# osmocom/osmo-trx

Measured on AMD Instinct MI355X. Metric: Mbursts/s detect+demod (156.25 sym, 4 SPS), higher is better.
Workload: dtype f32

## Files before the change

osmo_trx_amd/csrc/trx_kernel_nb.hip:

```cpp
#include "trx_k4_common.h"
#include "trx_nb_asm.inc"

#define NB_D_LEN    160
#define NB_CZ_LEN   (TRX_CZ_PAD + TRX_CORR_NARROW + TRX_CZ_PAD)
#define NB_SLICE    (K4_XS + NB_D_LEN + NB_CZ_LEN)
#define NB_COMP_ROWS (TRX_DELAY_FILTS + 1)
#define NB_TABLES_FLOATS (TRX_SINCV_LDS + 16 * WAVE + NB_COMP_ROWS * 36 + 16 + 8 * 8 + 5 * WAVE + 5 * WAVE + 2 * 8 * 16)
#define NB_TABLES_BYTES (NB_TABLES_FLOATS * 4)
#define NB_WPB 16
#define NB_POOL_RING 64
#define NB_POOL_UNSET (-1)
#define NB_POOL_END (-2)
#define NB_NO_BURST 0xffffffffu
#define NB_LDS_TAIL (16 + 4 * NB_POOL_RING)
#define NB_LDS_BYTES (NB_TABLES_BYTES + NB_WPB * NB_SLICE * 8 + NB_LDS_TAIL)
#define NB_MAX_TOA 32



typedef float v3f __attribute__((ext_vector_type(3)));
typedef int v4i __attribute__((ext_vector_type(4)));

template <typename T>
__device__ __forceinline__ unsigned lds_addr(const T *p)
{
	return (unsigned)(uintptr_t)(const __attribute__((address_space(3))) T *)p;
}

__global__ void __launch_bounds__(NB_WPB * WAVE)
nb_pull4_kernel(const uint32_t *__restrict__ iq, const trxhip_burst_params *__restrict__ params,
		trxhip_burst_result *__restrict__ results, float *__restrict__ soft, const trx_tables *__restrict__ tab,
		unsigned n_bursts, float thresh, float full_scale, unsigned *__restrict__ pool_ctr, unsigned *__restrict__ redo,
		float gk5, float gk6, float gk7, float gk8)
{
	static_assert(NB_TABLES_BYTES % 16 == 0 && (NB_SLICE * 8) % 16 == 0 && (K4_XS * 8) % 16 == 0 && (NB_D_LEN * 8) % 16 == 0, "16-byte LDS accesses");
	static_assert(NB_LDS_BYTES <= 160 * 1024, "LDS");
	static_assert(NB_ASM_GDEC_OFF == (TRX_SINCV_LDS + 16 * WAVE + NB_COMP_ROWS * 36) * 4, "tools/gen_nb_asm.py: LDS offset of the decimator taps");
	static_assert(NB_ASM_DEC_MAX_NACT == 15 + NB_ASM_CORR_MAX_LEN, "tools/gen_nb_asm.py: DEC and CORR change form at the same window");
	static_assert(NB_ASM_LSEQ_OFF == (NB_TABLES_FLOATS - 2 * 8 * 16) * 4, "tools/gen_nb_asm.py: LDS offset of the training-sequence taps");
	constexpr int NLD = 10;
	extern __shared__ __attribute__((aligned(16))) char smem[];
	const int lane0 = threadIdx.x & (WAVE - 1);
	const int wave = uni((int)(threadIdx.x >> 6));

	float *const sincv = reinterpret_cast<float *>(smem);
	float *const wa4f = sincv + TRX_SINCV_LDS;
	const float4 *const wa4 = reinterpret_cast<const float4 *>(wa4f);
	float *const comp = wa4f + 16 * WAVE;
	float *const gdec = comp + NB_COMP_ROWS * 36;
	float *const lhdr = gdec + 16;
	int *const pkcl = reinterpret_cast<int *>(lhdr + 8 * 8);
	int *const lcn = pkcl + 5 * WAVE;
	c32 *const lseq = reinterpret_cast<c32 *>(lcn + 5 * WAVE);
	c32 *const wbase = reinterpret_cast<c32 *>(smem + NB_TABLES_BYTES) + (size_t)wave * NB_SLICE;
	int *const wg_next = reinterpret_cast<int *>(reinterpret_cast<c32 *>(smem + NB_TABLES_BYTES) + (size_t)NB_WPB * NB_SLICE);
	int *const pool_g = wg_next + 4;
	c32 *const P = wbase;
	c32 *const D = wbase + K4_XS;
	c32 *const cz = D + NB_D_LEN + TRX_CZ_PAD;

	for (int i = threadIdx.x; i < TRX_SINCV_LDS; i += blockDim.x)
		sincv[i] = (i < TRX_SINCV_LEN) ? tab->sincv[i] : 0.0f;
	for (int i = threadIdx.x; i < 16 * WAVE; i += blockDim.x) {
		const int l = i & (WAVE - 1), u = i >> 6;
		const PeakConst pcl = peak_const(l);
		const int q = (u < 8) ? pcl.loA + 512 * (7 - u) : pcl.hiA + 512 * (u - 8);
		wa4f[((u >> 2) * WAVE + l) * 4 + (u & 3)] = (q < TRX_SINCV_LEN) ? tab->sincv[q] : 0.0f;
	}
	for (int i = threadIdx.x; i < NB_COMP_ROWS * 36; i += blockDim.x) {
		const int f = i / 36, j = i % 36;
		comp[i] = (j >= TRX_FUSED_SH) ? tab->comp_filt[f][j - TRX_FUSED_SH] : 0.0f;
	}
	if (threadIdx.x < 16)
		gdec[threadIdx.x] = tab->dec_taps[threadIdx.x];
	if (threadIdx.x < 128)
		lseq[threadIdx.x] = make_float2(tab->seq[TRX_SEQ_TSC0 + (threadIdx.x >> 4)].taps[threadIdx.x & 15].re,
						tab->seq[TRX_SEQ_TSC0 + (threadIdx.x >> 4)].taps[threadIdx.x & 15].im);
	if (threadIdx.x < 64)
		lhdr[threadIdx.x] = reinterpret_cast<const float *>(&tab->seq[TRX_SEQ_TSC0 + (threadIdx.x >> 3)].gain)[threadIdx.x & 7];
	if (threadIdx.x < WAVE) {
		const PeakConst pc0 = peak_const(threadIdx.x);
		pkcl[0 * WAVE + threadIdx.x] = pc0.flA;
		pkcl[1 * WAVE + threadIdx.x] = pc0.loA;
		pkcl[2 * WAVE + threadIdx.x] = pc0.hiA;
		pkcl[3 * WAVE + threadIdx.x] = pc0.offB;
		pkcl[4 * WAVE + threadIdx.x] = pc0.ratio_off;
		lcn[0 * WAVE + threadIdx.x] = pc0.ratio_off * 8;
		lcn[1 * WAVE + threadIdx.x] = (pc0.flA - 8) * 8;
		lcn[2 * WAVE + threadIdx.x] = pc0.offB;
		const int l = threadIdx.x, e = (l - 52) / 3, t = (l - 52) % 3;
		const bool sp = l >= 52;
		lcn[3 * WAVE + l] = 8 * (sp ? (t == 0 ? e : t == 1 ? e + 3 : e - 3) : 4 + 3 * (l < 49 ? l : 49));
		lcn[4 * WAVE + l] = sp ? (e + (t == 2 ? 4 : 0)) * K4_NTP * 4 : -1;
	}
	for (int i = lane0; i < NB_SLICE; i += WAVE)
		wbase[i] = make_float2(0.0f, 0.0f);
	if (threadIdx.x == 0) {
		wg_next[0] = NB_WPB;
		wg_next[1] = 0;
	}
	if (threadIdx.x < NB_POOL_RING)
		pool_g[threadIdx.x] = NB_POOL_UNSET;
	__syncthreads();

	const float fs_db = 6.02059991f * __log2f(full_scale);
	const float thr2 = thresh * thresh;
	const float gc0 = thr2 * 1.0001e-5f;
	int t5pk = 0;
	bool t5_ok = true;
	for (int t = 0; t < 8; t++) {
		const int v = (int)(lhdr[8 * t + 5] * 512.0f);
		t5_ok = t5_ok && v >= -8 && v <= 7 && (float)v == lhdr[8 * t + 5] * 512.0f;
		t5pk |= (v & 15) << (4 * t);
	}
	t5pk = uni(t5pk);
	const unsigned long long e8_addr = reinterpret_cast<unsigned long long>(&tab->edge8[0][0][0]);
	const unsigned n_wg = gridDim.x;
	const unsigned n_groups = (n_bursts + 15u) >> 4;
	const bool pooled = pool_ctr != nullptr;
	const unsigned n_static_groups = pooled ? ((n_groups - (n_groups >> 3)) / n_wg) * n_wg : n_groups;
	const unsigned n_pool_groups = n_groups - n_static_groups;
	const unsigned gq = n_static_groups / n_wg, gr = n_static_groups % n_wg;
	const unsigned my_groups = gq + (blockIdx.x < gr ? 1u : 0u);
	const unsigned base16 = (blockIdx.x * gq + (blockIdx.x < gr ? blockIdx.x : gr)) << 4;
	unsigned items = my_groups << 4;
	if (base16 + items > n_bursts)
		items = (base16 < n_bursts) ? n_bursts - base16 : 0u;
	auto burst_of = [&](unsigned jj) -> unsigned {
		if (jj < items)
			return base16 + jj;
		if (!pooled)
			return NB_NO_BURST;
		const unsigned k = (jj - items) >> 4;
		volatile int *slot = pool_g + (k & (NB_POOL_RING - 1));
		int g;
		while ((g = *slot) == NB_POOL_UNSET)
			__builtin_amdgcn_s_sleep(2);
		g = uni(g);
		if (g < 0)
			return NB_NO_BURST;
		const unsigned bb = ((n_static_groups + (unsigned)g) << 4) + (jj & 15u);
		return bb < n_bursts ? bb : NB_NO_BURST;
	};
	auto pool_draw = [&](unsigned jj, bool ended, int lane) {
		const unsigned k = (jj + 16u - items) >> 4;
		int g = NB_POOL_END;
		if (!ended) {
			unsigned p = 0;
			if (lane == 0)
				p = __hip_atomic_fetch_add(pool_ctr, 1u, __ATOMIC_RELAXED, __HIP_MEMORY_SCOPE_AGENT);
			p = (unsigned)uni((int)p);
			g = (p < n_pool_groups) ? (int)p : NB_POOL_END;
		}
		if (lane == 0) {
			pool_g[(k + NB_POOL_RING / 2) & (NB_POOL_RING - 1)] = NB_POOL_UNSET;
			pool_g[k & (NB_POOL_RING - 1)] = g;
		}
	};

	uint32_t pre_i[NLD];
	uint32_t pre_prm = 0u;
	auto prefetch = [&](unsigned bb, int lane) {
		pre_prm = reinterpret_cast<const uint32_t *>(params)[2 * (size_t)bb];
		const uint32_t *src = iq + (size_t)bb * 625;
		const unsigned ul = (unsigned)lane & 63u;
#pragma unroll
		for (int r = 0; r < NLD - 1; r++)
			pre_i[r] = __builtin_nontemporal_load(src + (unsigned)(r * WAVE) + ul);
		pre_i[NLD - 1] = __builtin_nontemporal_load(src + (unsigned)((NLD - 1) * WAVE) + min(ul, 48u));
	};
	const unsigned b_first = burst_of((unsigned)wave);
	if (b_first != NB_NO_BURST)
		prefetch(b_first, lane0);

	v3f o = { 0.0f, 0.0f, 0.0f };
	int recw = 0;
	bool pend_any = false;
	bool pend_rec = false;
	unsigned pend_b = 0;
	bool left_any = false;
	int q_xr = 0, q_xi = 0, q_es = 0, q_toa = 0, q_s = 0, q_fl = 0, q_b = 0;
	int q_n = 0;
	auto flush_records = [&](const int lane) {
		if (lane < q_n) {
			const float *const h = lhdr + 8 * (q_fl & 0xff);
			const float xr = __int_as_float(q_xr), xi = __int_as_float(q_xi);
			const float a0 = xr * h[2], a1 = xr * h[3], a2 = xi * h[3], a3 = xi * h[2];
			const float amp_re = a0 - a2, amp_im = a1 + a3;
			const float toa = (float)q_toa * 0.001953125f;
			const float energy = __int_as_float(q_es) * 0.0125f;
			const float rssi = fs_db - 3.01029996f * __log2f(energy);
			const float p2 = xi * xi + xr * xr;
			const float C = p2 * h[7];
			const float S = __int_as_float(q_s);
			const float ci = 3.0103f * __log2f(C * __builtin_amdgcn_rcpf(S - C));
			const v4i r0 = { 1, __float_as_int(toa), __float_as_int(amp_re), __float_as_int(amp_im) };
			const v4i r1 = { __float_as_int(ci), __float_as_int(energy), __float_as_int(rssi), q_fl };
			asm volatile("global_store_dwordx4 %0, %1, off\n\t"
				     "global_store_dwordx4 %0, %2, off offset:16\n\t"
				     "s_nop 1"
				     :: "v"(results + (unsigned)q_b), "v"(r0), "v"(r1) : "memory");
		}
		q_n = 0;
	};

	auto demod_general = [&](const int nk, const c32 ampv, const int lane) -> bool {
		constexpr int L = 625, nwrite = 148;
		c32 *const dec = D;
		const trx_tables *tabc = tab;
		asm volatile("" : "+s"(tabc));
		const int w = nk >> 7, fr = nk & 127;
		const int fidx = (fr >= 2) ? (fr >> 1) : TRX_DELAY_FILTS;
		const float ian = __builtin_amdgcn_rcpf(norm2(ampv));
		const c32 scale = make_float2(ampv.x * ian, -ampv.y * ian);
		const int n_lo = w > 0 ? w : 0;
		const int n_hi = (L - 1 + w < 623) ? L - 1 + w : 623;
		const int i_full_lo = cdiv4(n_lo + 15), i_full_hi = fdiv4(n_hi);
		const int i0l = cdiv4(n_lo), i0h = i_full_hi + 1;
		const bool need_lo = (n_hi >= n_lo) && (i0l < i_full_lo) && (i0l < nwrite);
		const bool need_hi = (n_hi >= n_lo) && (i0h <= fdiv4(n_hi + 15)) && (i0h < nwrite);
		const bool lo_tab = need_lo && (n_hi >= 4 * (i_full_lo - 1));
		float ct0 = 0.0f, ct1 = 0.0f, ct2 = 0.0f;
		const int le = lane >> 4, lt = lane & 15;
		const int li = i0l + le;
		const int lt0 = n_lo + 15 - 4 * li;
		const bool lact = lt0 >= 1;
		if (lo_tab) {
			const float *row = &tabc->edge_lo[fidx][(lact ? lt0 : 1) - 1][lt];
			ct0 = row[0];
			ct1 = row[16];
			ct2 = (lt < 4) ? row[32] : 0.0f;
		}
		const bool hi_tab = need_hi && (w <= -2) && (n_lo <= 4 * i0h - 15);
		if ((need_lo && !lo_tab) || (need_hi && !hi_tab))
			return false;
		float ch0 = 0.0f, ch1 = 0.0f, ch2 = 0.0f;
		const int hi_i = i0h + le;
		const int htm = n_hi + 15 - 4 * hi_i;
		const bool hact = htm >= 0;
		if (hi_tab) {
			const float *row = &tabc->edge_hi[fidx][hact ? htm : 0][lt];
			ch0 = row[0];
			ch1 = row[16];
			ch2 = (lt < 4) ? row[32] : 0.0f;
		}
		{
			const int c_full = -24 - w;
			const int i_min = cdiv4(-36 - c_full), i_max = fdiv4(L + 1 - c_full);
			int ic = 3 * lane;
			if (ic < i_min) ic = i_min;
			if (ic > i_max - 2) ic = i_max - 2;
			v2f acc[3];
			asm volatile(NB_ASM_FIRG
				     : [a0] "=&v"(acc[0]), [a1] "=&v"(acc[1]), [a2] "=&v"(acc[2])
				     : [nk] "s"(nk), [pb] "s"(lds_addr(P)), [cb] "s"(lds_addr(comp) + 4u * (K4_U0 + TRX_FUSED_SH)), [kic] "v"(8 * ic)
				     : NB_ASM_CLOBBERS);
			if (n_lo == 0 && lo_tab && i_full_hi >= nwrite - 1) {
				if (lane < 52) {
#pragma unroll
					for (int j = 0; j < 3; j++)
						dec[3 * lane + j] = cmul(make_float2(acc[j].x, acc[j].y), scale);
				}
			} else {
#pragma unroll
				for (int j = 0; j < 3; j++) {
					const int i = 3 * lane + j;
					const bool full = (i >= i_full_lo) && (i <= i_full_hi);
					const c32 d = full ? cmul(make_float2(acc[j].x, acc[j].y), scale) : make_float2(0.0f, 0.0f);
					if (i < 156)
						dec[i] = d;
				}
			}
		}
		if (lo_tab) {
			const int s0 = 4 * li - 24 - w + lt;
			const c32 *pp = P + ((s0 & 3) * PH_A + PH_M0 + (s0 >> 2));
			const c32 x0 = lds_c32(pp), x1 = lds_c32(pp + 4), x2 = lds_c32(pp + 8);
			float ar = x0.x * ct0, ai = x0.y * ct0;
			ar = fmaf(x1.x, ct1, ar); ai = fmaf(x1.y, ct1, ai);
			ar = fmaf(x2.x, ct2, ar); ai = fmaf(x2.y, ct2, ai);
			const float sr = row_sum(ar), si = row_sum(ai);
			if (lt == 0 && lact)
				dec[li] = cmul(make_float2(sr, si), scale);
		}
		if (hi_tab) {
			const int s0 = 4 * hi_i - 24 - w + lt;
			const c32 *pp = P + ((s0 & 3) * PH_A + PH_M0 + (s0 >> 2));
			const c32 x0 = lds_c32(pp), x1 = lds_c32(pp + 4), x2 = lds_c32(pp + 8);
			float ar = x0.x * ch0, ai = x0.y * ch0;
			ar = fmaf(x1.x, ch1, ar); ai = fmaf(x1.y, ch1, ai);
			ar = fmaf(x2.x, ch2, ar); ai = fmaf(x2.y, ch2, ai);
			const float sr = row_sum(ar), si = row_sum(ai);
			if (lt == 0 && hact && hi_i < 156)
				dec[hi_i] = cmul(make_float2(sr, si), scale);
		}
		wave_sync();
		auto pick = [&](int i) {
			const float d = reinterpret_cast<const float *>(dec + i)[i & 1];
			return __builtin_amdgcn_fmed3f(fmaf((i & 2) ? -0.5f : 0.5f, d, 0.5f), 0.0f, 1.0f);
		};
		const bool reg = lane >= 2 && lane < 50;
		const int i0 = reg ? 3 * lane - 2 : ((((lane - 54) * 11) >> 5) & 3);
		o.x = pick(i0);
		o.y = pick(reg ? i0 + 1 : 0);
		o.z = pick(reg ? i0 + 2 : 0);
		wave_sync();
		return true;
	};

	DIAG_DECL;
	unsigned j_next = 0, b_next = NB_NO_BURST;
	for (unsigned b = b_first; b != NB_NO_BURST; b = b_next) {
		int lane;
		asm volatile("v_mbcnt_lo_u32_b32 %0, -1, 0\n\tv_mbcnt_hi_u32_b32 %0, -1, %0" : "=v"(lane));
		const int ticket = claim_issue(wg_next);
		const unsigned prm0 = (unsigned)uni((int)pre_prm);
		const unsigned max_toa = prm0 >> 16;
		const int tsc = (prm0 >> 8) & 0xff;
		bool leave = ((prm0 & 0xf8ffu) != (unsigned)TRXHIP_TSC) || (max_toa > NB_MAX_TOA) || !t5_ok;

		c32 *const pload = P + (lane & 3) * PH_A + PH_M0 + (lane >> 2);
		float amax = 0.0f, epart = 0.0f;
#ifdef TRX_DIAG
		DIAG_MARK(12);
		asm volatile("s_waitcnt vmcnt(0)" ::: "memory");
		DIAG_MARK(13);
#endif
		if (!leave) {
#pragma unroll
			for (int r = 0; r < NLD; r++) {
				const int i = r * WAVE + lane;
				if (r < NLD - 1 || i < 625) {
					const c32 v = make_float2((float)(int16_t)(pre_i[r] & 0xffffu), (float)(int16_t)(pre_i[r] >> 16));
					pload[16 * r] = v;
					asm("v_max3_f32 %0, %0, |%1|, |%2|" : "+v"(amax) : "v"(v.x), "v"(v.y));
					if (r < 5)
						epart = fmaf(v.x, v.x, fmaf(v.y, v.y, epart));
				}
			}
		} else {
#pragma unroll
			for (int r = 0; r < NLD; r++)
				asm volatile("" :: "v"(pre_i[r]));
		}
		DIAG_MARK(14);
		if (pend_any) {
			float *const so = soft + (size_t)pend_b * 148;
			int *const rp = reinterpret_cast<int *>(results + pend_b);
			const float oe = o.x;
			asm volatile("s_bfm_b64 exec, 48, 2\n\t"
				     "global_store_dwordx3 %0, %1, %2 offset:16\n\t"
				     "s_mov_b32 exec_lo, 0\n\t"
			     "s_mov_b32 exec_hi, 0x92400000\n\t"
				     "global_store_dword %3, %4, %2\n\t"
				     "s_mov_b64 exec, %8\n\t"
				     "global_store_dword %5, %6, %7\n\t"
				     "s_mov_b64 exec, -1\n\t"
				     "s_nop 0"
				     :: "v"((lane - 2) * 12), "v"(o), "s"(so), "v"((((lane - 54) * 11) >> 5) * 4), "v"(oe), "v"(lane * 4), "v"(recw), "s"(rp),
				        "s"(pend_rec ? 0xffull : 0ull)
				     : "memory");
		}
		pend_any = false;
		DIAG_MARK(16);
		j_next = (unsigned)(leave ? claim_take(ticket) : claim_take_behind<5>(ticket));
		b_next = burst_of(j_next);
		if (pooled && (j_next & 15u) == 0u && j_next + 16u >= items)
			pool_draw(j_next, b_next == NB_NO_BURST && j_next >= items, lane);
		DIAG_MARK(17);
		if (b_next != NB_NO_BURST)
			prefetch(b_next, lane);
		DIAG_MARK(15);

		int clip = 0;
		if (!leave) {
			clip = __ballot(amax > TRX_CLIP_THRESH) != 0ull;

			const int len = 16 + (int)max_toa;
			__builtin_assume(len >= 16 && len <= 16 + NB_MAX_TOA);
			const unsigned vd_addr = lds_addr(D) + 8u * (unsigned)lane, vcz_addr = lds_addr(cz) + 8u * (unsigned)lane;
			unsigned long long bad;
			float dr, di;
			asm volatile(NB_ASM_DEC
				     : [bad] "=s"(bad), [dr] "=&v"(dr), [di] "=&v"(di)
				     : [pd] "v"(lds_addr(P + PH_M0 + 52) + 8u * (unsigned)lane), [vd] "v"(vd_addr), [vd4] "v"(vd_addr - 32u), [zero] "v"(0),
				       [nact] "s"(15 + len)
				     : NB_ASM_CLOBBERS);
			DIAG_MARK(2);
			{
				float v;
				const int lag0 = (len <= NB_ASM_CORR_MAX_LEN) ? NB_ASM_CORR_LANE0 : 0;
				asm volatile(NB_ASM_CORR
					     : [nrm] "=&v"(v)
					     : [vd] "v"(vd_addr), [vcz] "v"(vcz_addr), [vdm] "v"(vd_addr - 8u * NB_ASM_CORR_LANE0),
					       [vczm] "v"(vcz_addr - 8u * NB_ASM_CORR_LANE0), [dr] "v"(dr), [di] "v"(di), [len] "s"(len), [tsc] "s"(tsc), [bad] "s"(bad)
					     : NB_ASM_CLOBBERS);
				DIAG_MARK(3);
				int m_bits, es_bits, bidx;
				int kr, ka, kb, kic, ktp;
				asm volatile(NB_ASM_AMAX("ds_read_b32 %[kr], %[l4] offset:%c[lc]", "ds_read_b32 %[ka], %[l4] offset:%c[lc]+256",
							 "ds_read_b32 %[kb], %[l4] offset:%c[lc]+512", "ds_read_b32 %[kic], %[l4] offset:%c[lc]+768",
							 "ds_read_b32 %[ktp], %[l4] offset:%c[lc]+1024", "s_nop 0", "s_nop 0", "s_nop 0")
					     "s_sub_u32 %[bidx], %[bidx], %[lag0]\n\t"
					     "s_waitcnt lgkmcnt(0)"
					     : [m] "=&s"(m_bits), [es] "=&s"(es_bits), [bidx] "=&s"(bidx), [kr] "=&v"(kr), [ka] "=&v"(ka), [kb] "=&v"(kb),
					       [kic] "=&v"(kic), [ktp] "=&v"(ktp)
					     : [nrm] "v"(v), [ep] "v"(epart), [l4] "v"(4 * lane), [lag0] "s"(lag0),
					       [lc] "n"((TRX_SINCV_LDS + 16 * WAVE + NB_COMP_ROWS * 36 + 16 + 64 + 5 * WAVE) * 4)
					     : NB_ASM_CLOBBERS);
				DIAG_MARK(4);
				int hit = 0;
				int toa512 = 0;
				if (m_bits != 0) {
					int st, e512;
					float km;
					asm volatile(NB_ASM_DETA
						     : [st] "=&s"(st), [e] "=&s"(e512), [km] "=&v"(km)
						     : [bidx] "s"(bidx), [len] "s"(len), [czb] "s"(lds_addr(cz)), [kr] "v"(kr), [ka] "v"(ka), [l16] "v"(16 * lane),
						       [k5] "s"(gk5), [k6] "s"(gk6), [k7] "s"(gk7), [k8] "s"(gk8), [c0] "v"(gc0)
						     : NB_ASM_CLOBBERS);
					DIAG_MARK(5);
					int xr_bits = 0, xi_bits = 0;
					if (st == 1) {
						asm volatile(NB_ASM_DETB
							     : [st] "=&s"(st), [toa] "=&s"(toa512), [xr] "=&s"(xr_bits), [xi] "=&s"(xi_bits)
							     : [e] "s"(e512), [kb] "v"(kb), [czb] "s"(lds_addr(cz)), [km] "v"(km)
							     : NB_ASM_CLOBBERS);
						DIAG_MARK(6);
					}
					if (st == 3) {
						if (lane == 0)
							atomicAdd(&g_trx_fast_stats[0], 1ull);
						PeakConst pkc;
						pkc.flA = pkcl[0 * WAVE + lane]; pkc.loA = pkcl[1 * WAVE + lane]; pkc.hiA = pkcl[2 * WAVE + lane];
						pkc.offB = pkcl[3 * WAVE + lane]; pkc.ratio_off = pkcl[4 * WAVE + lane];
						c32 xcorr;
						peak_detect_spec(cz, bidx, sincv, pkc, lane, &toa512, &xcorr, wa4);
						toa512 = uni(toa512);
						xr_bits = uni(__float_as_int(xcorr.x));
						xi_bits = uni(__float_as_int(xcorr.y));
						st = 1;
					}
					if (st == 2) {
						leave = true;
						if (lane == 0) atomicAdd(&g_trx_fast_stats[2], 1ull);
					}
					if (st == 1) {
						hit = 1;
						int ok, s_bits;
						float d0, d1, d2;
						const int t5 = (t5pk << (28 - 4 * tsc)) >> 28;
						asm volatile("s_setprio 0");
						asm volatile(NB_ASM_TAIL
							     : [ok] "=&s"(ok), [ssum] "=&s"(s_bits), [d0] "=&v"(d0), [d1] "=&v"(d1), [d2] "=&v"(d2)
							     : [toa] "s"(toa512), [xr] "s"(xr_bits), [xi] "s"(xi_bits), [t5] "s"(t5), [hdrb] "s"(lds_addr(lhdr) + 32u * (unsigned)tsc),
							       [e8lo] "s"((unsigned)e8_addr), [e8hi] "s"((unsigned)(e8_addr >> 32)), [l16] "v"(16 * lane),
							       [vd] "v"(vd_addr), [pb] "s"(lds_addr(P)), [cb] "s"(lds_addr(comp) + 4u * (K4_U0 + TRX_FUSED_SH)), [db] "s"(lds_addr(D)),
							       [kic] "v"(kic), [ktp] "v"(ktp)
							     : NB_ASM_CLOBBERS);
						DIAG_MARK(10);
						asm volatile("s_setprio 2");
						if (!ok) {
							if (lane == 0) atomicAdd(&g_trx_fast_stats[3], 1ull);
							const float *const h = lhdr + 8 * tsc;
							const float xr = __int_as_float(xr_bits), xi = __int_as_float(xi_bits);
							const float a0 = xr * h[2], a1 = xr * h[3], a2 = xi * h[3], a3 = xi * h[2];
							const c32 ampv = make_float2(unif(a0 - a2), unif(a1 + a3));
							if (!demod_general(t5 + 10 * 512 - toa512, ampv, lane))
								leave = true;
						}
						if (!leave) {
							asm("s_lshl_b64 exec, 1, %[n]\n\t"
						    "v_mov_b32_e32 %[qxr], %[xr]\n\t"
						    "v_mov_b32_e32 %[qxi], %[xi]\n\t"
						    "v_mov_b32_e32 %[qes], %[es]\n\t"
						    "v_mov_b32_e32 %[qtoa], %[toa]\n\t"
						    "v_mov_b32_e32 %[qs], %[ss]\n\t"
						    "v_mov_b32_e32 %[qfl], %[fl]\n\t"
						    "v_mov_b32_e32 %[qb], %[b]\n\t"
						    "s_mov_b64 exec, -1"
						    : [qxr] "+v"(q_xr), [qxi] "+v"(q_xi), [qes] "+v"(q_es), [qtoa] "+v"(q_toa), [qs] "+v"(q_s), [qfl] "+v"(q_fl),
						      [qb] "+v"(q_b)
						    : [n] "s"(uni(q_n)), [xr] "s"(xr_bits), [xi] "s"(xi_bits), [es] "s"(es_bits), [toa] "s"(toa512 - t5 - 10 * 512),
						      [ss] "s"(s_bits), [fl] "s"((int)((uint32_t)tsc | ((uint32_t)clip << 8) | (37u << 24))), [b] "s"((int)b));
						q_n++;
						}
						if (ok) {
							o.x = __builtin_amdgcn_fmed3f(fmaf(0.5f, d0, 0.5f), 0.0f, 1.0f);
							o.y = __builtin_amdgcn_fmed3f(fmaf(0.5f, d1, 0.5f), 0.0f, 1.0f);
							o.z = __builtin_amdgcn_fmed3f(fmaf(0.5f, d2, 0.5f), 0.0f, 1.0f);
						}
					}
				}
				if (!hit && !leave) {
					const float energy = __int_as_float(es_bits) * 0.0125f;
					const float rssi = fs_db - 3.01029996f * __log2f(energy);
					const uint32_t flags = ((uint32_t)clip << 8) | (1u << 16);
					int word = clip ? -TRXHIP_SIGERR_CLIP : 0;
					word = put_lane<1>(word, 0.0f);
					word = put_lane<2>(word, 0.0f);
					word = put_lane<3>(word, 0.0f);
					word = put_lane<4>(word, 0.0f);
					word = put_lane<5>(word, energy);
					word = put_lane<6>(word, rssi);
					word = write_lane<7>(word, (int)flags);
					recw = word;
					o = (v3f){ 0.0f, 0.0f, 0.0f };
				}
				pend_rec = !hit;
			}
		}
		if (leave) {
			if (lane == 0) {
				reinterpret_cast<uint8_t *>(redo + TRX_REDO_HDR)[b] = 1;
				if (!left_any)
					__hip_atomic_store(redo, 1u, __ATOMIC_RELAXED, __HIP_MEMORY_SCOPE_AGENT);
			}
			left_any = true;
			continue;
		}
		pend_b = b;
		pend_any = true;
		if (q_n == WAVE)
			flush_records(lane);
		DIAG_MARK(11);
	}
	if (pend_any) {
		int lane;
		asm volatile("v_mbcnt_lo_u32_b32 %0, -1, 0\n\tv_mbcnt_hi_u32_b32 %0, -1, %0" : "=v"(lane));
		float *const so = soft + (size_t)pend_b * 148;
		int *const rp = reinterpret_cast<int *>(results + pend_b);
		const float oe = o.x;
		asm volatile("s_bfm_b64 exec, 48, 2\n\t"
			     "global_store_dwordx3 %0, %1, %2 offset:16\n\t"
		     "s_mov_b32 exec_lo, 0\n\t"
		     "s_mov_b32 exec_hi, 0x92400000\n\t"
			     "global_store_dword %3, %4, %2\n\t"
			     "s_mov_b64 exec, %8\n\t"
			     "global_store_dword %5, %6, %7\n\t"
			     "s_mov_b64 exec, -1\n\t"
			     "s_nop 0"
			     :: "v"((lane - 2) * 12), "v"(o), "s"(so), "v"((((lane - 54) * 11) >> 5) * 4), "v"(oe), "v"(lane * 4), "v"(recw), "s"(rp),
			        "s"(pend_rec ? 0xffull : 0ull)
			     : "memory");
	}
	{
		int lane;
		asm volatile("v_mbcnt_lo_u32_b32 %0, -1, 0\n\tv_mbcnt_hi_u32_b32 %0, -1, %0" : "=v"(lane));
		flush_records(lane);
	}
	DIAG_FLUSH();
	if (pooled) {
		__syncthreads();
		int tid0;
		asm volatile("v_mbcnt_lo_u32_b32 %0, -1, 0\n\tv_mbcnt_hi_u32_b32 %0, -1, %0" : "=v"(tid0));
		if (tid0 == 0 && atomicAdd(wg_next + 1, 1) == 0) {
			const unsigned d = __hip_atomic_fetch_add(pool_ctr + 1, 1u, __ATOMIC_ACQ_REL, __HIP_MEMORY_SCOPE_AGENT);
			if (d == gridDim.x - 1u) {
				__hip_atomic_store(pool_ctr, 0u, __ATOMIC_RELAXED, __HIP_MEMORY_SCOPE_AGENT);
				__hip_atomic_store(pool_ctr + 1, 0u, __ATOMIC_RELEASE, __HIP_MEMORY_SCOPE_AGENT);
			}
		}
	}
}
```

osmo_trx_amd/csrc/trx_nb_asm.inc:

```
#define NB_ASM_GDEC_OFF 29968
#define NB_ASM_LSEQ_OFF 32848
#define NB_ASM_DEC_MAX_NACT 60
#define NB_ASM_CORR_LANE0 19
#define NB_ASM_CORR_MAX_LEN 45
#define NB_ASM_CLOBBERS "v64", "v65", "v66", "v67", "v68", "v69", "v70", "v71", "v72", "v73", "v74", "v75", "v76", "v77", "v78", "v79", "v80", "v81", "v82", "v83", "v84", "v85", "v86", "v87", "v88", "v89", "v90", "v91", "v92", "v93", "v94", "v95", "v96", "v97", "v98", "v99", "v100", "v101", "v102", "v103", "v104", "v105", "v106", "v107", "v108", "v109", "v110", "v111", "v112", "v113", "v114", "v115", "v116", "v117", "v118", "v119", "v120", "v121", "v122", "v123", "v124", "v125", "v126", "v127", "s87", "s88", "s89", "s90", "s91", "s92", "s93", "s94", "s95", "s96", "s97", "s98", "s99", "vcc", "scc", "memory"
#define NB_ASM_DEC \
	"s_cmp_gt_u32 %[nact], 60\n\t" \
	"s_cbranch_scc1 .Lnb_dec_wide\n\t" \
	"s_sub_u32 s88, 60, %[nact]\n\t" \
	"s_lshr_b64 exec, -1, s88\n\t" \
	"ds_read_b128 v[120:123], %[zero] offset:29968\n\t" \
	"ds_read_b128 v[124:127], %[zero] offset:29984\n\t" \
	"ds_read_b64 v[98:99], %[pd] offset:1440\n\t" \
	"ds_read_b64 v[100:101], %[pd] offset:2880\n\t" \
	"ds_read_b64 v[102:103], %[pd] offset:4320\n\t" \
	"ds_read_b64 v[96:97], %[pd] offset:0\n\t" \
	"s_waitcnt lgkmcnt(3)\n\t" \
	"v_pk_mul_f32 v[64:65], v[98:99], v[120:121] op_sel:[0,0] op_sel_hi:[1,0]\n\t" \
	"s_waitcnt lgkmcnt(2)\n\t" \
	"v_pk_mul_f32 v[66:67], v[100:101], v[120:121] op_sel:[0,1] op_sel_hi:[1,1]\n\t" \
	"s_waitcnt lgkmcnt(1)\n\t" \
	"v_pk_mul_f32 v[68:69], v[102:103], v[122:123] op_sel:[0,0] op_sel_hi:[1,0]\n\t" \
	"v_pk_add_f32 v[104:105], v[64:65], v[66:67]\n\t" \
	"s_waitcnt lgkmcnt(0)\n\t" \
	"v_pk_mul_f32 v[70:71], v[96:97], v[122:123] op_sel:[0,1] op_sel_hi:[1,1]\n\t" \
	"v_pk_add_f32 v[104:105], v[104:105], v[68:69]\n\t" \
	"v_pk_mul_f32 v[72:73], v[98:99], v[124:125] op_sel:[0,0] op_sel_hi:[1,0]\n\t" \
	"v_pk_mul_f32 v[74:75], v[100:101], v[124:125] op_sel:[0,1] op_sel_hi:[1,1]\n\t" \
	"v_add_f32_dpp v104, v104, v70 wave_shr:1 row_mask:0xf bank_mask:0xf bound_ctrl:0\n\t" \
	"v_add_f32_dpp v105, v105, v71 wave_shr:1 row_mask:0xf bank_mask:0xf bound_ctrl:0\n\t" \
	"v_pk_mul_f32 v[76:77], v[102:103], v[126:127] op_sel:[0,0] op_sel_hi:[1,0]\n\t" \
	"v_pk_add_f32 v[104:105], v[104:105], v[72:73]\n\t" \
	"v_pk_mul_f32 v[78:79], v[96:97], v[126:127] op_sel:[0,1] op_sel_hi:[1,1]\n\t" \
	"v_pk_add_f32 v[104:105], v[104:105], v[74:75]\n\t" \
	"v_pk_mul_f32 v[80:81], v[98:99], v[126:127] op_sel:[0,1] op_sel_hi:[1,1]\n\t" \
	"v_pk_add_f32 v[104:105], v[104:105], v[76:77]\n\t" \
	"v_pk_mul_f32 v[82:83], v[100:101], v[126:127] op_sel:[0,0] op_sel_hi:[1,0]\n\t" \
	"v_pk_mul_f32 v[84:85], v[102:103], v[124:125] op_sel:[0,1] op_sel_hi:[1,1]\n\t" \
	"v_add_f32_dpp v104, v104, v78 wave_shr:1 row_mask:0xf bank_mask:0xf bound_ctrl:0\n\t" \
	"v_add_f32_dpp v105, v105, v79 wave_shr:1 row_mask:0xf bank_mask:0xf bound_ctrl:0\n\t" \
	"v_pk_mul_f32 v[86:87], v[96:97], v[124:125] op_sel:[0,0] op_sel_hi:[1,0]\n\t" \
	"v_pk_add_f32 v[104:105], v[104:105], v[80:81]\n\t" \
	"v_pk_mul_f32 v[88:89], v[98:99], v[122:123] op_sel:[0,1] op_sel_hi:[1,1]\n\t" \
	"v_pk_add_f32 v[104:105], v[104:105], v[82:83]\n\t" \
	"v_pk_mul_f32 v[90:91], v[100:101], v[122:123] op_sel:[0,0] op_sel_hi:[1,0]\n\t" \
	"v_pk_add_f32 v[104:105], v[104:105], v[84:85]\n\t" \
	"v_pk_mul_f32 v[92:93], v[102:103], v[120:121] op_sel:[0,1] op_sel_hi:[1,1]\n\t" \
	"v_pk_mul_f32 v[94:95], v[96:97], v[120:121] op_sel:[0,0] op_sel_hi:[1,0]\n\t" \
	"v_add_f32_dpp v104, v104, v86 wave_shr:1 row_mask:0xf bank_mask:0xf bound_ctrl:0\n\t" \
	"v_add_f32_dpp v105, v105, v87 wave_shr:1 row_mask:0xf bank_mask:0xf bound_ctrl:0\n\t" \
	"v_pk_add_f32 v[104:105], v[104:105], v[88:89]\n\t" \
	"s_nop 0\n\t" \
	"v_pk_add_f32 v[104:105], v[104:105], v[90:91]\n\t" \
	"s_nop 0\n\t" \
	"v_pk_add_f32 v[104:105], v[104:105], v[92:93]\n\t" \
	"s_nop 1\n\t" \
	"v_add_f32_dpp %[dr], v104, v94 wave_shr:1 row_mask:0xf bank_mask:0xf bound_ctrl:0\n\t" \
	"v_add_f32_dpp %[di], v105, v95 wave_shr:1 row_mask:0xf bank_mask:0xf bound_ctrl:0\n\t" \
	"s_bfm_b64 exec, %[nact], 4\n\t" \
	"ds_write2_b32 %[vd4], %[dr], %[di] offset1:1\n\t" \
	"v_min_f32_e64 v106, |%[dr]|, |%[di]|\n\t" \
	"v_max_f32_e64 v107, |%[dr]|, |%[di]|\n\t" \
	"v_ldexp_f32 v106, v106, 17\n\t" \
	"v_cmp_lt_f32_e32 vcc, v106, v107\n\t" \
	"s_mov_b64 exec, -1\n\t" \
	"s_mov_b64 %[bad], vcc\n\t" \
	"s_waitcnt lgkmcnt(0)\n\t" \
	"s_branch .Lnb_dec_end\n\t" \
	".Lnb_dec_wide:\n\t" \
	"s_bfm_b64 exec, %[nact], 0\n\t" \
	"ds_read_b128 v[120:123], %[zero] offset:29968\n\t" \
	"ds_read_b128 v[124:127], %[zero] offset:29984\n\t" \
	"ds_read_b64 v[88:89], %[pd] offset:1440\n\t" \
	"ds_read_b64 v[90:91], %[pd] offset:2880\n\t" \
	"ds_read_b64 v[92:93], %[pd] offset:4320\n\t" \
	"ds_read_b64 v[94:95], %[pd] offset:8\n\t" \
	"ds_read_b64 v[96:97], %[pd] offset:1448\n\t" \
	"ds_read_b64 v[98:99], %[pd] offset:2888\n\t" \
	"ds_read_b64 v[100:101], %[pd] offset:4328\n\t" \
	"ds_read_b64 v[102:103], %[pd] offset:16\n\t" \
	"ds_read_b64 v[104:105], %[pd] offset:1456\n\t" \
	"ds_read_b64 v[106:107], %[pd] offset:2896\n\t" \
	"ds_read_b64 v[108:109], %[pd] offset:4336\n\t" \
	"ds_read_b64 v[110:111], %[pd] offset:24\n\t" \
	"ds_read_b64 v[112:113], %[pd] offset:1464\n\t" \
	"ds_read_b64 v[114:115], %[pd] offset:2904\n\t" \
	"ds_read_b64 v[116:117], %[pd] offset:4344\n\t" \
	"ds_read_b64 v[118:119], %[pd] offset:32\n\t" \
	"s_waitcnt lgkmcnt(12)\n\t" \
	"v_pk_mul_f32 v[88:89], v[88:89], v[120:121] op_sel:[0,0] op_sel_hi:[1,0]\n\t" \
	"v_pk_mul_f32 v[90:91], v[90:91], v[120:121] op_sel:[0,1] op_sel_hi:[1,1]\n\t" \
	"v_pk_mul_f32 v[92:93], v[92:93], v[122:123] op_sel:[0,0] op_sel_hi:[1,0]\n\t" \
	"v_pk_add_f32 v[88:89], v[88:89], v[90:91]\n\t" \
	"v_pk_mul_f32 v[94:95], v[94:95], v[122:123] op_sel:[0,1] op_sel_hi:[1,1]\n\t" \
	"v_pk_add_f32 v[88:89], v[88:89], v[92:93]\n\t" \
	"s_waitcnt lgkmcnt(8)\n\t" \
	"v_pk_mul_f32 v[96:97], v[96:97], v[124:125] op_sel:[0,0] op_sel_hi:[1,0]\n\t" \
	"v_pk_add_f32 v[88:89], v[88:89], v[94:95]\n\t" \
	"v_pk_mul_f32 v[98:99], v[98:99], v[124:125] op_sel:[0,1] op_sel_hi:[1,1]\n\t" \
	"v_pk_add_f32 v[88:89], v[88:89], v[96:97]\n\t" \
	"v_pk_mul_f32 v[100:101], v[100:101], v[126:127] op_sel:[0,0] op_sel_hi:[1,0]\n\t" \
	"v_pk_add_f32 v[88:89], v[88:89], v[98:99]\n\t" \
	"v_pk_mul_f32 v[102:103], v[102:103], v[126:127] op_sel:[0,1] op_sel_hi:[1,1]\n\t" \
	"v_pk_add_f32 v[88:89], v[88:89], v[100:101]\n\t" \
	"s_waitcnt lgkmcnt(4)\n\t" \
	"v_pk_mul_f32 v[104:105], v[104:105], v[126:127] op_sel:[0,1] op_sel_hi:[1,1]\n\t" \
	"v_pk_add_f32 v[88:89], v[88:89], v[102:103]\n\t" \
	"v_pk_mul_f32 v[106:107], v[106:107], v[126:127] op_sel:[0,0] op_sel_hi:[1,0]\n\t" \
	"v_pk_add_f32 v[88:89], v[88:89], v[104:105]\n\t" \
	"v_pk_mul_f32 v[108:109], v[108:109], v[124:125] op_sel:[0,1] op_sel_hi:[1,1]\n\t" \
	"v_pk_add_f32 v[88:89], v[88:89], v[106:107]\n\t" \
	"v_pk_mul_f32 v[110:111], v[110:111], v[124:125] op_sel:[0,0] op_sel_hi:[1,0]\n\t" \
	"v_pk_add_f32 v[88:89], v[88:89], v[108:109]\n\t" \
	"s_waitcnt lgkmcnt(0)\n\t" \
	"v_pk_mul_f32 v[112:113], v[112:113], v[122:123] op_sel:[0,1] op_sel_hi:[1,1]\n\t" \
	"v_pk_add_f32 v[88:89], v[88:89], v[110:111]\n\t" \
	"v_pk_mul_f32 v[114:115], v[114:115], v[122:123] op_sel:[0,0] op_sel_hi:[1,0]\n\t" \
	"v_pk_add_f32 v[88:89], v[88:89], v[112:113]\n\t" \
	"v_pk_mul_f32 v[116:117], v[116:117], v[120:121] op_sel:[0,1] op_sel_hi:[1,1]\n\t" \
	"v_pk_add_f32 v[88:89], v[88:89], v[114:115]\n\t" \
	"v_pk_mul_f32 v[118:119], v[118:119], v[120:121] op_sel:[0,0] op_sel_hi:[1,0]\n\t" \
	"v_pk_add_f32 v[88:89], v[88:89], v[116:117]\n\t" \
	"s_nop 0\n\t" \
	"v_pk_add_f32 v[88:89], v[88:89], v[118:119]\n\t" \
	"ds_write_b64 %[vd], v[88:89]\n\t" \
	"v_min_f32_e64 v90, |v88|, |v89|\n\t" \
	"v_max_f32_e64 v91, |v88|, |v89|\n\t" \
	"v_ldexp_f32 v90, v90, 17\n\t" \
	"v_cmp_lt_f32_e32 vcc, v90, v91\n\t" \
	"s_mov_b64 exec, -1\n\t" \
	"s_mov_b64 %[bad], vcc\n\t" \
	"s_waitcnt lgkmcnt(0)\n\t" \
	".Lnb_dec_end:\n\t"
#define NB_ASM_CORR \
	"s_cmp_gt_u32 %[len], 45\n\t" \
	"s_cbranch_scc1 .Lnb_corr_wide\n\t" \
	"v_mov_b64_e32 v[120:121], 0\n\t" \
	"v_mov_b64_e32 v[122:123], 0\n\t" \
	"v_mov_b32_e32 %[nrm], 0\n\t" \
	"s_lshl_b32 s90, %[len], 3\n\t" \
	"s_sub_u32 s91, 45, %[len]\n\t" \
	"v_add_u32_e32 v64, s90, %[vcz]\n\t" \
	"s_lshr_b64 exec, -1, s91\n\t" \
	"s_cmp_lg_u64 %[bad], 0\n\t" \
	"s_cbranch_scc1 .Lnb_corrr_mul\n\t" \
	"s_getpc_b64 s[88:89]\n\t" \
	".Lnb_corrr_pc:\n\t" \
	"s_mul_i32 s90, %[tsc], .Lnb_corrr_v1-.Lnb_corrr_v0\n\t" \
	"s_add_u32 s88, s88, s90\n\t" \
	"s_addc_u32 s89, s89, 0\n\t" \
	"s_add_u32 s88, s88, .Lnb_corrr_v0-.Lnb_corrr_pc\n\t" \
	"s_addc_u32 s89, s89, 0\n\t" \
	"s_setpc_b64 s[88:89]\n\t" \
	".Lnb_corrr_v0:\n\t" \
	"v_sub_f32_e32 v120, 0, %[dr]\n\t" \
	"v_sub_f32_e32 v121, 0, %[di]\n\t" \
	"s_nop 0\n\t" \
	"v_add_f32_dpp v120, v120, %[di] wave_shr:1 row_mask:0xf bank_mask:0xf bound_ctrl:0\n\t" \
	"v_sub_f32_dpp v121, v121, %[dr] wave_shr:1 row_mask:0xf bank_mask:0xf bound_ctrl:0\n\t" \
	"s_nop 0\n\t" \
	"v_add_f32_dpp v120, v120, %[dr] wave_shr:1 row_mask:0xf bank_mask:0xf bound_ctrl:0\n\t" \
	"v_add_f32_dpp v121, v121, %[di] wave_shr:1 row_mask:0xf bank_mask:0xf bound_ctrl:0\n\t" \
	"s_nop 0\n\t" \
	"v_add_f32_dpp v120, v120, %[di] wave_shr:1 row_mask:0xf bank_mask:0xf bound_ctrl:0\n\t" \
	"v_sub_f32_dpp v121, v121, %[dr] wave_shr:1 row_mask:0xf bank_mask:0xf bound_ctrl:0\n\t" \
	"s_nop 0\n\t" \
	"v_sub_f32_dpp v120, v120, %[dr] wave_shr:1 row_mask:0xf bank_mask:0xf bound_ctrl:0\n\t" \
	"v_sub_f32_dpp v121, v121, %[di] wave_shr:1 row_mask:0xf bank_mask:0xf bound_ctrl:0\n\t" \
	"s_nop 0\n\t" \
	"v_add_f32_dpp v120, v120, %[di] wave_shr:1 row_mask:0xf bank_mask:0xf bound_ctrl:0\n\t" \
	"v_sub_f32_dpp v121, v121, %[dr] wave_shr:1 row_mask:0xf bank_mask:0xf bound_ctrl:0\n\t" \
	"s_nop 0\n\t" \
	"v_sub_f32_dpp v120, v120, %[dr] wave_shr:1 row_mask:0xf bank_mask:0xf bound_ctrl:0\n\t" \
	"v_sub_f32_dpp v121, v121, %[di] wave_shr:1 row_mask:0xf bank_mask:0xf bound_ctrl:0\n\t" \
	"s_nop 0\n\t" \
	"v_sub_f32_dpp v120, v120, %[di] wave_shr:1 row_mask:0xf bank_mask:0xf bound_ctrl:0\n\t" \
	"v_add_f32_dpp v121, v121, %[dr] wave_shr:1 row_mask:0xf bank_mask:0xf bound_ctrl:0\n\t" \
	"s_nop 0\n\t" \
	"v_add_f32_dpp v120, v120, %[dr] wave_shr:1 row_mask:0xf bank_mask:0xf bound_ctrl:0\n\t" \
	"v_add_f32_dpp v121, v121, %[di] wave_shr:1 row_mask:0xf bank_mask:0xf bound_ctrl:0\n\t" \
	"s_nop 0\n\t" \
	"v_sub_f32_dpp v120, v120, %[di] wave_shr:1 row_mask:0xf bank_mask:0xf bound_ctrl:0\n\t" \
	"v_add_f32_dpp v121, v121, %[dr] wave_shr:1 row_mask:0xf bank_mask:0xf bound_ctrl:0\n\t" \
	"s_nop 0\n\t" \
	"v_sub_f32_dpp v120, v120, %[dr] wave_shr:1 row_mask:0xf bank_mask:0xf bound_ctrl:0\n\t" \
	"v_sub_f32_dpp v121, v121, %[di] wave_shr:1 row_mask:0xf bank_mask:0xf bound_ctrl:0\n\t" \
	"s_nop 0\n\t" \
	"v_sub_f32_dpp v120, v120, %[di] wave_shr:1 row_mask:0xf bank_mask:0xf bound_ctrl:0\n\t" \
	"v_add_f32_dpp v121, v121, %[dr] wave_shr:1 row_mask:0xf bank_mask:0xf bound_ctrl:0\n\t" \
	"s_nop 0\n\t" \
	"v_add_f32_dpp v120, v120, %[dr] wave_shr:1 row_mask:0xf bank_mask:0xf bound_ctrl:0\n\t" \
	"v_add_f32_dpp v121, v121, %[di] wave_shr:1 row_mask:0xf bank_mask:0xf bound_ctrl:0\n\t" \
	"s_nop 0\n\t" \
	"v_sub_f32_dpp v120, v120, %[di] wave_shr:1 row_mask:0xf bank_mask:0xf bound_ctrl:0\n\t" \
	"v_add_f32_dpp v121, v121, %[dr] wave_shr:1 row_mask:0xf bank_mask:0xf bound_ctrl:0\n\t" \
	"s_nop 0\n\t" \
	"v_sub_f32_dpp v120, v120, %[dr] wave_shr:1 row_mask:0xf bank_mask:0xf bound_ctrl:0\n\t" \
	"v_sub_f32_dpp v121, v121, %[di] wave_shr:1 row_mask:0xf bank_mask:0xf bound_ctrl:0\n\t" \
	"s_nop 0\n\t" \
	"v_sub_f32_dpp v120, v120, %[di] wave_shr:1 row_mask:0xf bank_mask:0xf bound_ctrl:0\n\t" \
	"v_add_f32_dpp v121, v121, %[dr] wave_shr:1 row_mask:0xf bank_mask:0xf bound_ctrl:0\n\t" \
	"s_branch .Lnb_corrr_join\n\t" \
	".Lnb_corrr_v1:\n\t" \
	"v_sub_f32_e32 v120, 0, %[dr]\n\t" \
	"v_sub_f32_e32 v121, 0, %[di]\n\t" \
	"s_nop 0\n\t" \
	"v_add_f32_dpp v120, v120, %[di] wave_shr:1 row_mask:0xf bank_mask:0xf bound_ctrl:0\n\t" \
	"v_sub_f32_dpp v121, v121, %[dr] wave_shr:1 row_mask:0xf bank_mask:0xf bound_ctrl:0\n\t" \
	"s_nop 0\n\t" \
	"v_add_f32_dpp v120, v120, %[dr] wave_shr:1 row_mask:0xf bank_mask:0xf bound_ctrl:0\n\t" \
	"v_add_f32_dpp v121, v121, %[di] wave_shr:1 row_mask:0xf bank_mask:0xf bound_ctrl:0\n\t" \
	"s_nop 0\n\t" \
	"v_add_f32_dpp v120, v120, %[di] wave_shr:1 row_mask:0xf bank_mask:0xf bound_ctrl:0\n\t" \
	"v_sub_f32_dpp v121, v121, %[dr] wave_shr:1 row_mask:0xf bank_mask:0xf bound_ctrl:0\n\t" \
	"s_nop 0\n\t" \
	"v_sub_f32_dpp v120, v120, %[dr] wave_shr:1 row_mask:0xf bank_mask:0xf bound_ctrl:0\n\t" \
	"v_sub_f32_dpp v121, v121, %[di] wave_shr:1 row_mask:0xf bank_mask:0xf bound_ctrl:0\n\t" \
	"s_nop 0\n\t" \
	"v_add_f32_dpp v120, v120, %[di] wave_shr:1 row_mask:0xf bank_mask:0xf bound_ctrl:0\n\t" \
	"v_sub_f32_dpp v121, v121, %[dr] wave_shr:1 row_mask:0xf bank_mask:0xf bound_ctrl:0\n\t" \
	"s_nop 0\n\t" \
	"v_add_f32_dpp v120, v120, %[dr] wave_shr:1 row_mask:0xf bank_mask:0xf bound_ctrl:0\n\t" \
	"v_add_f32_dpp v121, v121, %[di] wave_shr:1 row_mask:0xf bank_mask:0xf bound_ctrl:0\n\t" \
	"s_nop 0\n\t" \
	"v_add_f32_dpp v120, v120, %[di] wave_shr:1 row_mask:0xf bank_mask:0xf bound_ctrl:0\n\t" \
	"v_sub_f32_dpp v121, v121, %[dr] wave_shr:1 row_mask:0xf bank_mask:0xf bound_ctrl:0\n\t" \
	"s_nop 0\n\t" \
	"v_sub_f32_dpp v120, v120, %[dr] wave_shr:1 row_mask:0xf bank_mask:0xf bound_ctrl:0\n\t" \
	"v_sub_f32_dpp v121, v121, %[di] wave_shr:1 row_mask:0xf bank_mask:0xf bound_ctrl:0\n\t" \
	"s_nop 0\n\t" \
	"v_sub_f32_dpp v120, v120, %[di] wave_shr:1 row_mask:0xf bank_mask:0xf bound_ctrl:0\n\t" \
	"v_add_f32_dpp v121, v121, %[dr] wave_shr:1 row_mask:0xf bank_mask:0xf bound_ctrl:0\n\t" \
	"s_nop 0\n\t" \
	"v_sub_f32_dpp v120, v120, %[dr] wave_shr:1 row_mask:0xf bank_mask:0xf bound_ctrl:0\n\t" \
	"v_sub_f32_dpp v121, v121, %[di] wave_shr:1 row_mask:0xf bank_mask:0xf bound_ctrl:0\n\t" \
	"s_nop 0\n\t" \
	"v_sub_f32_dpp v120, v120, %[di] wave_shr:1 row_mask:0xf bank_mask:0xf bound_ctrl:0\n\t" \
	"v_add_f32_dpp v121, v121, %[dr] wave_shr:1 row_mask:0xf bank_mask:0xf bound_ctrl:0\n\t" \
	"s_nop 0\n\t" \
	"v_add_f32_dpp v120, v120, %[dr] wave_shr:1 row_mask:0xf bank_mask:0xf bound_ctrl:0\n\t" \
	"v_add_f32_dpp v121, v121, %[di] wave_shr:1 row_mask:0xf bank_mask:0xf bound_ctrl:0\n\t" \
	"s_nop 0\n\t" \
	"v_sub_f32_dpp v120, v120, %[di] wave_shr:1 row_mask:0xf bank_mask:0xf bound_ctrl:0\n\t" \
	"v_add_f32_dpp v121, v121, %[dr] wave_shr:1 row_mask:0xf bank_mask:0xf bound_ctrl:0\n\t" \
	"s_nop 0\n\t" \
	"v_sub_f32_dpp v120, v120, %[dr] wave_shr:1 row_mask:0xf bank_mask:0xf bound_ctrl:0\n\t" \
	"v_sub_f32_dpp v121, v121, %[di] wave_shr:1 row_mask:0xf bank_mask:0xf bound_ctrl:0\n\t" \
	"s_nop 0\n\t" \
	"v_add_f32_dpp v120, v120, %[di] wave_shr:1 row_mask:0xf bank_mask:0xf bound_ctrl:0\n\t" \
	"v_sub_f32_dpp v121, v121, %[dr] wave_shr:1 row_mask:0xf bank_mask:0xf bound_ctrl:0\n\t" \
	"s_branch .Lnb_corrr_join\n\t" \
	".Lnb_corrr_v2:\n\t" \
	"v_add_f32_e32 v120, 0, %[dr]\n\t" \
	"v_add_f32_e32 v121, 0, %[di]\n\t" \
	"s_nop 0\n\t" \
	"v_sub_f32_dpp v120, v120, %[di] wave_shr:1 row_mask:0xf bank_mask:0xf bound_ctrl:0\n\t" \
	"v_add_f32_dpp v121, v121, %[dr] wave_shr:1 row_mask:0xf bank_mask:0xf bound_ctrl:0\n\t" \
	"s_nop 0\n\t" \
	"v_add_f32_dpp v120, v120, %[dr] wave_shr:1 row_mask:0xf bank_mask:0xf bound_ctrl:0\n\t" \
	"v_add_f32_dpp v121, v121, %[di] wave_shr:1 row_mask:0xf bank_mask:0xf bound_ctrl:0\n\t" \
	"s_nop 0\n\t" \
	"v_add_f32_dpp v120, v120, %[di] wave_shr:1 row_mask:0xf bank_mask:0xf bound_ctrl:0\n\t" \
	"v_sub_f32_dpp v121, v121, %[dr] wave_shr:1 row_mask:0xf bank_mask:0xf bound_ctrl:0\n\t" \
	"s_nop 0\n\t" \
	"v_add_f32_dpp v120, v120, %[dr] wave_shr:1 row_mask:0xf bank_mask:0xf bound_ctrl:0\n\t" \
	"v_add_f32_dpp v121, v121, %[di] wave_shr:1 row_mask:0xf bank_mask:0xf bound_ctrl:0\n\t" \
	"s_nop 0\n\t" \
	"v_sub_f32_dpp v120, v120, %[di] wave_shr:1 row_mask:0xf bank_mask:0xf bound_ctrl:0\n\t" \
	"v_add_f32_dpp v121, v121, %[dr] wave_shr:1 row_mask:0xf bank_mask:0xf bound_ctrl:0\n\t" \
	"s_nop 0\n\t" \
	"v_add_f32_dpp v120, v120, %[dr] wave_shr:1 row_mask:0xf bank_mask:0xf bound_ctrl:0\n\t" \
	"v_add_f32_dpp v121, v121, %[di] wave_shr:1 row_mask:0xf bank_mask:0xf bound_ctrl:0\n\t" \
	"s_nop 0\n\t" \
	"v_add_f32_dpp v120, v120, %[di] wave_shr:1 row_mask:0xf bank_mask:0xf bound_ctrl:0\n\t" \
	"v_sub_f32_dpp v121, v121, %[dr] wave_shr:1 row_mask:0xf bank_mask:0xf bound_ctrl:0\n\t" \
	"s_nop 0\n\t" \
	"v_add_f32_dpp v120, v120, %[dr] wave_shr:1 row_mask:0xf bank_mask:0xf bound_ctrl:0\n\t" \
	"v_add_f32_dpp v121, v121, %[di] wave_shr:1 row_mask:0xf bank_mask:0xf bound_ctrl:0\n\t" \
	"s_nop 0\n\t" \
	"v_sub_f32_dpp v120, v120, %[di] wave_shr:1 row_mask:0xf bank_mask:0xf bound_ctrl:0\n\t" \
	"v_add_f32_dpp v121, v121, %[dr] wave_shr:1 row_mask:0xf bank_mask:0xf bound_ctrl:0\n\t" \
	"s_nop 0\n\t" \
	"v_sub_f32_dpp v120, v120, %[dr] wave_shr:1 row_mask:0xf bank_mask:0xf bound_ctrl:0\n\t" \
	"v_sub_f32_dpp v121, v121, %[di] wave_shr:1 row_mask:0xf bank_mask:0xf bound_ctrl:0\n\t" \
	"s_nop 0\n\t" \
	"v_sub_f32_dpp v120, v120, %[di] wave_shr:1 row_mask:0xf bank_mask:0xf bound_ctrl:0\n\t" \
	"v_add_f32_dpp v121, v121, %[dr] wave_shr:1 row_mask:0xf bank_mask:0xf bound_ctrl:0\n\t" \
	"s_nop 0\n\t" \
	"v_sub_f32_dpp v120, v120, %[dr] wave_shr:1 row_mask:0xf bank_mask:0xf bound_ctrl:0\n\t" \
	"v_sub_f32_dpp v121, v121, %[di] wave_shr:1 row_mask:0xf bank_mask:0xf bound_ctrl:0\n\t" \
	"s_nop 0\n\t" \
	"v_add_f32_dpp v120, v120, %[di] wave_shr:1 row_mask:0xf bank_mask:0xf bound_ctrl:0\n\t" \
	"v_sub_f32_dpp v121, v121, %[dr] wave_shr:1 row_mask:0xf bank_mask:0xf bound_ctrl:0\n\t" \
	"s_nop 0\n\t" \
	"v_sub_f32_dpp v120, v120, %[dr] wave_shr:1 row_mask:0xf bank_mask:0xf bound_ctrl:0\n\t" \
	"v_sub_f32_dpp v121, v121, %[di] wave_shr:1 row_mask:0xf bank_mask:0xf bound_ctrl:0\n\t" \
	"s_nop 0\n\t" \
	"v_sub_f32_dpp v120, v120, %[di] wave_shr:1 row_mask:0xf bank_mask:0xf bound_ctrl:0\n\t" \
	"v_add_f32_dpp v121, v121, %[dr] wave_shr:1 row_mask:0xf bank_mask:0xf bound_ctrl:0\n\t" \
	"s_branch .Lnb_corrr_join\n\t" \
	".Lnb_corrr_v3:\n\t" \
	"v_sub_f32_e32 v120, 0, %[dr]\n\t" \
	"v_sub_f32_e32 v121, 0, %[di]\n\t" \
	"s_nop 0\n\t" \
	"v_sub_f32_dpp v120, v120, %[di] wave_shr:1 row_mask:0xf bank_mask:0xf bound_ctrl:0\n\t" \
	"v_add_f32_dpp v121, v121, %[dr] wave_shr:1 row_mask:0xf bank_mask:0xf bound_ctrl:0\n\t" \
	"s_nop 0\n\t" \
// ... 494 lines not shown
	"s_waitcnt lgkmcnt(5)\n\t" \
	"v_pk_add_f32 v[120:121], v[120:121], v[108:109] neg_lo:[0,1] neg_hi:[0,1]\n\t" \
	"s_waitcnt lgkmcnt(4)\n\t" \
	"v_pk_add_f32 v[120:121], v[120:121], v[110:111] op_sel:[0,1] op_sel_hi:[1,0] neg_lo:[0,1] neg_hi:[0,0]\n\t" \
	"s_waitcnt lgkmcnt(3)\n\t" \
	"v_pk_add_f32 v[120:121], v[120:121], v[112:113] neg_lo:[0,1] neg_hi:[0,1]\n\t" \
	"s_waitcnt lgkmcnt(2)\n\t" \
	"v_pk_add_f32 v[120:121], v[120:121], v[114:115] op_sel:[0,1] op_sel_hi:[1,0] neg_lo:[0,0] neg_hi:[0,1]\n\t" \
	"s_waitcnt lgkmcnt(1)\n\t" \
	"v_pk_add_f32 v[120:121], v[120:121], v[116:117] neg_lo:[0,1] neg_hi:[0,1]\n\t" \
	"s_waitcnt lgkmcnt(0)\n\t" \
	"v_pk_add_f32 v[120:121], v[120:121], v[118:119] op_sel:[0,1] op_sel_hi:[1,0] neg_lo:[0,1] neg_hi:[0,0]\n\t" \
	"s_branch .Lnb_corrw_join\n\t" \
	".Lnb_corrw_v3:\n\t" \
	"s_waitcnt lgkmcnt(15)\n\t" \
	"v_pk_add_f32 v[120:121], v[120:121], v[88:89] neg_lo:[0,1] neg_hi:[0,1]\n\t" \
	"s_waitcnt lgkmcnt(14)\n\t" \
	"v_pk_add_f32 v[120:121], v[120:121], v[90:91] op_sel:[0,1] op_sel_hi:[1,0] neg_lo:[0,1] neg_hi:[0,0]\n\t" \
	"s_waitcnt lgkmcnt(13)\n\t" \
	"v_pk_add_f32 v[120:121], v[120:121], v[92:93]\n\t" \
	"s_waitcnt lgkmcnt(12)\n\t" \
	"v_pk_add_f32 v[120:121], v[120:121], v[94:95] op_sel:[0,1] op_sel_hi:[1,0] neg_lo:[0,0] neg_hi:[0,1]\n\t" \
	"s_waitcnt lgkmcnt(11)\n\t" \
	"v_pk_add_f32 v[120:121], v[120:121], v[96:97]\n\t" \
	"s_waitcnt lgkmcnt(10)\n\t" \
	"v_pk_add_f32 v[120:121], v[120:121], v[98:99] op_sel:[0,1] op_sel_hi:[1,0] neg_lo:[0,1] neg_hi:[0,0]\n\t" \
	"s_waitcnt lgkmcnt(9)\n\t" \
	"v_pk_add_f32 v[120:121], v[120:121], v[100:101]\n\t" \
	"s_waitcnt lgkmcnt(8)\n\t" \
	"v_pk_add_f32 v[120:121], v[120:121], v[102:103] op_sel:[0,1] op_sel_hi:[1,0] neg_lo:[0,1] neg_hi:[0,0]\n\t" \
	"s_waitcnt lgkmcnt(7)\n\t" \
	"v_pk_add_f32 v[120:121], v[120:121], v[104:105] neg_lo:[0,1] neg_hi:[0,1]\n\t" \
	"s_waitcnt lgkmcnt(6)\n\t" \
	"v_pk_add_f32 v[120:121], v[120:121], v[106:107] op_sel:[0,1] op_sel_hi:[1,0] neg_lo:[0,0] neg_hi:[0,1]\n\t" \
	"s_waitcnt lgkmcnt(5)\n\t" \
	"v_pk_add_f32 v[120:121], v[120:121], v[108:109] neg_lo:[0,1] neg_hi:[0,1]\n\t" \
	"s_waitcnt lgkmcnt(4)\n\t" \
	"v_pk_add_f32 v[120:121], v[120:121], v[110:111] op_sel:[0,1] op_sel_hi:[1,0] neg_lo:[0,1] neg_hi:[0,0]\n\t" \
	"s_waitcnt lgkmcnt(3)\n\t" \
	"v_pk_add_f32 v[120:121], v[120:121], v[112:113] neg_lo:[0,1] neg_hi:[0,1]\n\t" \
	"s_waitcnt lgkmcnt(2)\n\t" \
	"v_pk_add_f32 v[120:121], v[120:121], v[114:115] op_sel:[0,1] op_sel_hi:[1,0] neg_lo:[0,0] neg_hi:[0,1]\n\t" \
	"s_waitcnt lgkmcnt(1)\n\t" \
	"v_pk_add_f32 v[120:121], v[120:121], v[116:117] neg_lo:[0,1] neg_hi:[0,1]\n\t" \
	"s_waitcnt lgkmcnt(0)\n\t" \
	"v_pk_add_f32 v[120:121], v[120:121], v[118:119] op_sel:[0,1] op_sel_hi:[1,0] neg_lo:[0,1] neg_hi:[0,0]\n\t" \
	"s_branch .Lnb_corrw_join\n\t" \
	".Lnb_corrw_v4:\n\t" \
	"s_waitcnt lgkmcnt(15)\n\t" \
	"v_pk_add_f32 v[120:121], v[120:121], v[88:89]\n\t" \
	"s_waitcnt lgkmcnt(14)\n\t" \
	"v_pk_add_f32 v[120:121], v[120:121], v[90:91] op_sel:[0,1] op_sel_hi:[1,0] neg_lo:[0,1] neg_hi:[0,0]\n\t" \
	"s_waitcnt lgkmcnt(13)\n\t" \
	"v_pk_add_f32 v[120:121], v[120:121], v[92:93] neg_lo:[0,1] neg_hi:[0,1]\n\t" \
	"s_waitcnt lgkmcnt(12)\n\t" \
	"v_pk_add_f32 v[120:121], v[120:121], v[94:95] op_sel:[0,1] op_sel_hi:[1,0] neg_lo:[0,0] neg_hi:[0,1]\n\t" \
	"s_waitcnt lgkmcnt(11)\n\t" \
	"v_pk_add_f32 v[120:121], v[120:121], v[96:97] neg_lo:[0,1] neg_hi:[0,1]\n\t" \
	"s_waitcnt lgkmcnt(10)\n\t" \
	"v_pk_add_f32 v[120:121], v[120:121], v[98:99] op_sel:[0,1] op_sel_hi:[1,0] neg_lo:[0,1] neg_hi:[0,0]\n\t" \
	"s_waitcnt lgkmcnt(9)\n\t" \
	"v_pk_add_f32 v[120:121], v[120:121], v[100:101] neg_lo:[0,1] neg_hi:[0,1]\n\t" \
	"s_waitcnt lgkmcnt(8)\n\t" \
	"v_pk_add_f32 v[120:121], v[120:121], v[102:103] op_sel:[0,1] op_sel_hi:[1,0] neg_lo:[0,1] neg_hi:[0,0]\n\t" \
	"s_waitcnt lgkmcnt(7)\n\t" \
	"v_pk_add_f32 v[120:121], v[120:121], v[104:105] neg_lo:[0,1] neg_hi:[0,1]\n\t" \
	"s_waitcnt lgkmcnt(6)\n\t" \
	"v_pk_add_f32 v[120:121], v[120:121], v[106:107] op_sel:[0,1] op_sel_hi:[1,0] neg_lo:[0,0] neg_hi:[0,1]\n\t" \
	"s_waitcnt lgkmcnt(5)\n\t" \
	"v_pk_add_f32 v[120:121], v[120:121], v[108:109] neg_lo:[0,1] neg_hi:[0,1]\n\t" \
	"s_waitcnt lgkmcnt(4)\n\t" \
	"v_pk_add_f32 v[120:121], v[120:121], v[110:111] op_sel:[0,1] op_sel_hi:[1,0] neg_lo:[0,1] neg_hi:[0,0]\n\t" \
	"s_waitcnt lgkmcnt(3)\n\t" \
	"v_pk_add_f32 v[120:121], v[120:121], v[112:113]\n\t" \
	"s_waitcnt lgkmcnt(2)\n\t" \
	"v_pk_add_f32 v[120:121], v[120:121], v[114:115] op_sel:[0,1] op_sel_hi:[1,0] neg_lo:[0,0] neg_hi:[0,1]\n\t" \
	"s_waitcnt lgkmcnt(1)\n\t" \
	"v_pk_add_f32 v[120:121], v[120:121], v[116:117]\n\t" \
	"s_waitcnt lgkmcnt(0)\n\t" \
	"v_pk_add_f32 v[120:121], v[120:121], v[118:119] op_sel:[0,1] op_sel_hi:[1,0] neg_lo:[0,0] neg_hi:[0,1]\n\t" \
	"s_branch .Lnb_corrw_join\n\t" \
	".Lnb_corrw_v5:\n\t" \
	"s_waitcnt lgkmcnt(15)\n\t" \
	"v_pk_add_f32 v[120:121], v[120:121], v[88:89] neg_lo:[0,1] neg_hi:[0,1]\n\t" \
	"s_waitcnt lgkmcnt(14)\n\t" \
	"v_pk_add_f32 v[120:121], v[120:121], v[90:91] op_sel:[0,1] op_sel_hi:[1,0] neg_lo:[0,1] neg_hi:[0,0]\n\t" \
	"s_waitcnt lgkmcnt(13)\n\t" \
	"v_pk_add_f32 v[120:121], v[120:121], v[92:93] neg_lo:[0,1] neg_hi:[0,1]\n\t" \
	"s_waitcnt lgkmcnt(12)\n\t" \
	"v_pk_add_f32 v[120:121], v[120:121], v[94:95] op_sel:[0,1] op_sel_hi:[1,0] neg_lo:[0,0] neg_hi:[0,1]\n\t" \
	"s_waitcnt lgkmcnt(11)\n\t" \
	"v_pk_add_f32 v[120:121], v[120:121], v[96:97]\n\t" \
	"s_waitcnt lgkmcnt(10)\n\t" \
	"v_pk_add_f32 v[120:121], v[120:121], v[98:99] op_sel:[0,1] op_sel_hi:[1,0] neg_lo:[0,1] neg_hi:[0,0]\n\t" \
	"s_waitcnt lgkmcnt(9)\n\t" \
	"v_pk_add_f32 v[120:121], v[120:121], v[100:101]\n\t" \
	"s_waitcnt lgkmcnt(8)\n\t" \
	"v_pk_add_f32 v[120:121], v[120:121], v[102:103] op_sel:[0,1] op_sel_hi:[1,0] neg_lo:[0,1] neg_hi:[0,0]\n\t" \
	"s_waitcnt lgkmcnt(7)\n\t" \
	"v_pk_add_f32 v[120:121], v[120:121], v[104:105]\n\t" \
	"s_waitcnt lgkmcnt(6)\n\t" \
	"v_pk_add_f32 v[120:121], v[120:121], v[106:107] op_sel:[0,1] op_sel_hi:[1,0] neg_lo:[0,0] neg_hi:[0,1]\n\t" \
	"s_waitcnt lgkmcnt(5)\n\t" \
	"v_pk_add_f32 v[120:121], v[120:121], v[108:109] neg_lo:[0,1] neg_hi:[0,1]\n\t" \
	"s_waitcnt lgkmcnt(4)\n\t" \
	"v_pk_add_f32 v[120:121], v[120:121], v[110:111] op_sel:[0,1] op_sel_hi:[1,0] neg_lo:[0,1] neg_hi:[0,0]\n\t" \
	"s_waitcnt lgkmcnt(3)\n\t" \
	"v_pk_add_f32 v[120:121], v[120:121], v[112:113] neg_lo:[0,1] neg_hi:[0,1]\n\t" \
	"s_waitcnt lgkmcnt(2)\n\t" \
	"v_pk_add_f32 v[120:121], v[120:121], v[114:115] op_sel:[0,1] op_sel_hi:[1,0] neg_lo:[0,0] neg_hi:[0,1]\n\t" \
	"s_waitcnt lgkmcnt(1)\n\t" \
	"v_pk_add_f32 v[120:121], v[120:121], v[116:117] neg_lo:[0,1] neg_hi:[0,1]\n\t" \
	"s_waitcnt lgkmcnt(0)\n\t" \
	"v_pk_add_f32 v[120:121], v[120:121], v[118:119] op_sel:[0,1] op_sel_hi:[1,0] neg_lo:[0,0] neg_hi:[0,1]\n\t" \
	"s_branch .Lnb_corrw_join\n\t" \
	".Lnb_corrw_v6:\n\t" \
	"s_waitcnt lgkmcnt(15)\n\t" \
	"v_pk_add_f32 v[120:121], v[120:121], v[88:89] neg_lo:[0,1] neg_hi:[0,1]\n\t" \
	"s_waitcnt lgkmcnt(14)\n\t" \
	"v_pk_add_f32 v[120:121], v[120:121], v[90:91] op_sel:[0,1] op_sel_hi:[1,0] neg_lo:[0,1] neg_hi:[0,0]\n\t" \
	"s_waitcnt lgkmcnt(13)\n\t" \
	"v_pk_add_f32 v[120:121], v[120:121], v[92:93]\n\t" \
	"s_waitcnt lgkmcnt(12)\n\t" \
	"v_pk_add_f32 v[120:121], v[120:121], v[94:95] op_sel:[0,1] op_sel_hi:[1,0] neg_lo:[0,0] neg_hi:[0,1]\n\t" \
	"s_waitcnt lgkmcnt(11)\n\t" \
	"v_pk_add_f32 v[120:121], v[120:121], v[96:97] neg_lo:[0,1] neg_hi:[0,1]\n\t" \
	"s_waitcnt lgkmcnt(10)\n\t" \
	"v_pk_add_f32 v[120:121], v[120:121], v[98:99] op_sel:[0,1] op_sel_hi:[1,0] neg_lo:[0,0] neg_hi:[0,1]\n\t" \
	"s_waitcnt lgkmcnt(9)\n\t" \
	"v_pk_add_f32 v[120:121], v[120:121], v[100:101]\n\t" \
	"s_waitcnt lgkmcnt(8)\n\t" \
	"v_pk_add_f32 v[120:121], v[120:121], v[102:103] op_sel:[0,1] op_sel_hi:[1,0] neg_lo:[0,0] neg_hi:[0,1]\n\t" \
	"s_waitcnt lgkmcnt(7)\n\t" \
	"v_pk_add_f32 v[120:121], v[120:121], v[104:105]\n\t" \
	"s_waitcnt lgkmcnt(6)\n\t" \
	"v_pk_add_f32 v[120:121], v[120:121], v[106:107] op_sel:[0,1] op_sel_hi:[1,0] neg_lo:[0,0] neg_hi:[0,1]\n\t" \
	"s_waitcnt lgkmcnt(5)\n\t" \
	"v_pk_add_f32 v[120:121], v[120:121], v[108:109] neg_lo:[0,1] neg_hi:[0,1]\n\t" \
	"s_waitcnt lgkmcnt(4)\n\t" \
	"v_pk_add_f32 v[120:121], v[120:121], v[110:111] op_sel:[0,1] op_sel_hi:[1,0] neg_lo:[0,0] neg_hi:[0,1]\n\t" \
	"s_waitcnt lgkmcnt(3)\n\t" \
	"v_pk_add_f32 v[120:121], v[120:121], v[112:113]\n\t" \
	"s_waitcnt lgkmcnt(2)\n\t" \
	"v_pk_add_f32 v[120:121], v[120:121], v[114:115] op_sel:[0,1] op_sel_hi:[1,0] neg_lo:[0,1] neg_hi:[0,0]\n\t" \
	"s_waitcnt lgkmcnt(1)\n\t" \
	"v_pk_add_f32 v[120:121], v[120:121], v[116:117] neg_lo:[0,1] neg_hi:[0,1]\n\t" \
	"s_waitcnt lgkmcnt(0)\n\t" \
	"v_pk_add_f32 v[120:121], v[120:121], v[118:119] op_sel:[0,1] op_sel_hi:[1,0] neg_lo:[0,1] neg_hi:[0,0]\n\t" \
	"s_branch .Lnb_corrw_join\n\t" \
	".Lnb_corrw_v7:\n\t" \
	"s_waitcnt lgkmcnt(15)\n\t" \
	"v_pk_add_f32 v[120:121], v[120:121], v[88:89] neg_lo:[0,1] neg_hi:[0,1]\n\t" \
	"s_waitcnt lgkmcnt(14)\n\t" \
	"v_pk_add_f32 v[120:121], v[120:121], v[90:91] op_sel:[0,1] op_sel_hi:[1,0] neg_lo:[0,1] neg_hi:[0,0]\n\t" \
	"s_waitcnt lgkmcnt(13)\n\t" \
	"v_pk_add_f32 v[120:121], v[120:121], v[92:93]\n\t" \
	"s_waitcnt lgkmcnt(12)\n\t" \
	"v_pk_add_f32 v[120:121], v[120:121], v[94:95] op_sel:[0,1] op_sel_hi:[1,0] neg_lo:[0,1] neg_hi:[0,0]\n\t" \
	"s_waitcnt lgkmcnt(11)\n\t" \
	"v_pk_add_f32 v[120:121], v[120:121], v[96:97]\n\t" \
	"s_waitcnt lgkmcnt(10)\n\t" \
	"v_pk_add_f32 v[120:121], v[120:121], v[98:99] op_sel:[0,1] op_sel_hi:[1,0] neg_lo:[0,0] neg_hi:[0,1]\n\t" \
	"s_waitcnt lgkmcnt(9)\n\t" \
	"v_pk_add_f32 v[120:121], v[120:121], v[100:101]\n\t" \
	"s_waitcnt lgkmcnt(8)\n\t" \
	"v_pk_add_f32 v[120:121], v[120:121], v[102:103] op_sel:[0,1] op_sel_hi:[1,0] neg_lo:[0,1] neg_hi:[0,0]\n\t" \
	"s_waitcnt lgkmcnt(7)\n\t" \
	"v_pk_add_f32 v[120:121], v[120:121], v[104:105]\n\t" \
	"s_waitcnt lgkmcnt(6)\n\t" \
	"v_pk_add_f32 v[120:121], v[120:121], v[106:107] op_sel:[0,1] op_sel_hi:[1,0] neg_lo:[0,1] neg_hi:[0,0]\n\t" \
	"s_waitcnt lgkmcnt(5)\n\t" \
	"v_pk_add_f32 v[120:121], v[120:121], v[108:109] neg_lo:[0,1] neg_hi:[0,1]\n\t" \
	"s_waitcnt lgkmcnt(4)\n\t" \
	"v_pk_add_f32 v[120:121], v[120:121], v[110:111] op_sel:[0,1] op_sel_hi:[1,0] neg_lo:[0,0] neg_hi:[0,1]\n\t" \
	"s_waitcnt lgkmcnt(3)\n\t" \
	"v_pk_add_f32 v[120:121], v[120:121], v[112:113] neg_lo:[0,1] neg_hi:[0,1]\n\t" \
	"s_waitcnt lgkmcnt(2)\n\t" \
	"v_pk_add_f32 v[120:121], v[120:121], v[114:115] op_sel:[0,1] op_sel_hi:[1,0] neg_lo:[0,1] neg_hi:[0,0]\n\t" \
	"s_waitcnt lgkmcnt(1)\n\t" \
	"v_pk_add_f32 v[120:121], v[120:121], v[116:117] neg_lo:[0,1] neg_hi:[0,1]\n\t" \
	"s_waitcnt lgkmcnt(0)\n\t" \
	"v_pk_add_f32 v[120:121], v[120:121], v[118:119] op_sel:[0,1] op_sel_hi:[1,0] neg_lo:[0,0] neg_hi:[0,1]\n\t" \
	"s_branch .Lnb_corrw_join\n\t" \
	".Lnb_corrw_join:\n\t" \
	"s_add_u32 s90, %[len], 12\n\t" \
	"s_bfm_b64 exec, s90, 0\n\t" \
	"ds_write_b64 %[vcz], v[120:121]\n\t" \
	"s_mov_b64 exec, -1\n\t" \
	"v_pk_mul_f32 v[122:123], v[120:121], v[120:121]\n\t" \
	"s_waitcnt lgkmcnt(0)\n\t" \
	"v_add_f32_e32 %[nrm], v123, v122\n\t" \
	"s_branch .Lnb_corr_end\n\t" \
	".Lnb_corrw_mul:\n\t" \
	"s_lshl_b32 s90, %[tsc], 7\n\t" \
	"v_mov_b32_e32 v64, s90\n\t" \
	"ds_read_b128 v[66:69], v64 offset:32848\n\t" \
	"ds_read_b128 v[70:73], v64 offset:32864\n\t" \
	"ds_read_b128 v[74:77], v64 offset:32880\n\t" \
	"ds_read_b128 v[78:81], v64 offset:32896\n\t" \
	"s_waitcnt lgkmcnt(0)\n\t" \
	"v_pk_mul_f32 v[82:83], v[88:89], v[66:67] op_sel:[0,0] op_sel_hi:[0,1]\n\t" \
	"v_pk_mul_f32 v[84:85], v[88:89], v[66:67] op_sel:[1,1] op_sel_hi:[1,0]\n\t" \
	"s_nop 0\n\t" \
	"v_pk_add_f32 v[86:87], v[82:83], v[84:85] neg_lo:[0,1] neg_hi:[0,0]\n\t" \
	"s_nop 0\n\t" \
	"v_pk_add_f32 v[120:121], v[120:121], v[86:87]\n\t" \
	"v_pk_mul_f32 v[82:83], v[90:91], v[68:69] op_sel:[0,0] op_sel_hi:[0,1]\n\t" \
	"v_pk_mul_f32 v[84:85], v[90:91], v[68:69] op_sel:[1,1] op_sel_hi:[1,0]\n\t" \
	"s_nop 0\n\t" \
	"v_pk_add_f32 v[86:87], v[82:83], v[84:85] neg_lo:[0,1] neg_hi:[0,0]\n\t" \
	"s_nop 0\n\t" \
	"v_pk_add_f32 v[120:121], v[120:121], v[86:87]\n\t" \
	"v_pk_mul_f32 v[82:83], v[92:93], v[70:71] op_sel:[0,0] op_sel_hi:[0,1]\n\t" \
	"v_pk_mul_f32 v[84:85], v[92:93], v[70:71] op_sel:[1,1] op_sel_hi:[1,0]\n\t" \
	"s_nop 0\n\t" \
	"v_pk_add_f32 v[86:87], v[82:83], v[84:85] neg_lo:[0,1] neg_hi:[0,0]\n\t" \
	"s_nop 0\n\t" \
	"v_pk_add_f32 v[120:121], v[120:121], v[86:87]\n\t" \
	"v_pk_mul_f32 v[82:83], v[94:95], v[72:73] op_sel:[0,0] op_sel_hi:[0,1]\n\t" \
	"v_pk_mul_f32 v[84:85], v[94:95], v[72:73] op_sel:[1,1] op_sel_hi:[1,0]\n\t" \
	"s_nop 0\n\t" \
	"v_pk_add_f32 v[86:87], v[82:83], v[84:85] neg_lo:[0,1] neg_hi:[0,0]\n\t" \
	"s_nop 0\n\t" \
	"v_pk_add_f32 v[120:121], v[120:121], v[86:87]\n\t" \
	"v_pk_mul_f32 v[82:83], v[96:97], v[74:75] op_sel:[0,0] op_sel_hi:[0,1]\n\t" \
	"v_pk_mul_f32 v[84:85], v[96:97], v[74:75] op_sel:[1,1] op_sel_hi:[1,0]\n\t" \
	"s_nop 0\n\t" \
	"v_pk_add_f32 v[86:87], v[82:83], v[84:85] neg_lo:[0,1] neg_hi:[0,0]\n\t" \
	"s_nop 0\n\t" \
	"v_pk_add_f32 v[120:121], v[120:121], v[86:87]\n\t" \
	"v_pk_mul_f32 v[82:83], v[98:99], v[76:77] op_sel:[0,0] op_sel_hi:[0,1]\n\t" \
	"v_pk_mul_f32 v[84:85], v[98:99], v[76:77] op_sel:[1,1] op_sel_hi:[1,0]\n\t" \
	"s_nop 0\n\t" \
	"v_pk_add_f32 v[86:87], v[82:83], v[84:85] neg_lo:[0,1] neg_hi:[0,0]\n\t" \
	"s_nop 0\n\t" \
	"v_pk_add_f32 v[120:121], v[120:121], v[86:87]\n\t" \
	"v_pk_mul_f32 v[82:83], v[100:101], v[78:79] op_sel:[0,0] op_sel_hi:[0,1]\n\t" \
	"v_pk_mul_f32 v[84:85], v[100:101], v[78:79] op_sel:[1,1] op_sel_hi:[1,0]\n\t" \
	"s_nop 0\n\t" \
	"v_pk_add_f32 v[86:87], v[82:83], v[84:85] neg_lo:[0,1] neg_hi:[0,0]\n\t" \
	"s_nop 0\n\t" \
	"v_pk_add_f32 v[120:121], v[120:121], v[86:87]\n\t" \
	"v_pk_mul_f32 v[82:83], v[102:103], v[80:81] op_sel:[0,0] op_sel_hi:[0,1]\n\t" \
	"v_pk_mul_f32 v[84:85], v[102:103], v[80:81] op_sel:[1,1] op_sel_hi:[1,0]\n\t" \
	"s_nop 0\n\t" \
	"v_pk_add_f32 v[86:87], v[82:83], v[84:85] neg_lo:[0,1] neg_hi:[0,0]\n\t" \
	"s_nop 0\n\t" \
	"v_pk_add_f32 v[120:121], v[120:121], v[86:87]\n\t" \
	"ds_read_b128 v[66:69], v64 offset:32912\n\t" \
	"ds_read_b128 v[70:73], v64 offset:32928\n\t" \
	"ds_read_b128 v[74:77], v64 offset:32944\n\t" \
	"ds_read_b128 v[78:81], v64 offset:32960\n\t" \
	"s_waitcnt lgkmcnt(0)\n\t" \
	"v_pk_mul_f32 v[82:83], v[104:105], v[66:67] op_sel:[0,0] op_sel_hi:[0,1]\n\t" \
	"v_pk_mul_f32 v[84:85], v[104:105], v[66:67] op_sel:[1,1] op_sel_hi:[1,0]\n\t" \
	"s_nop 0\n\t" \
	"v_pk_add_f32 v[86:87], v[82:83], v[84:85] neg_lo:[0,1] neg_hi:[0,0]\n\t" \
	"s_nop 0\n\t" \
	"v_pk_add_f32 v[120:121], v[120:121], v[86:87]\n\t" \
	"v_pk_mul_f32 v[82:83], v[106:107], v[68:69] op_sel:[0,0] op_sel_hi:[0,1]\n\t" \
	"v_pk_mul_f32 v[84:85], v[106:107], v[68:69] op_sel:[1,1] op_sel_hi:[1,0]\n\t" \
	"s_nop 0\n\t" \
	"v_pk_add_f32 v[86:87], v[82:83], v[84:85] neg_lo:[0,1] neg_hi:[0,0]\n\t" \
	"s_nop 0\n\t" \
	"v_pk_add_f32 v[120:121], v[120:121], v[86:87]\n\t" \
	"v_pk_mul_f32 v[82:83], v[108:109], v[70:71] op_sel:[0,0] op_sel_hi:[0,1]\n\t" \
	"v_pk_mul_f32 v[84:85], v[108:109], v[70:71] op_sel:[1,1] op_sel_hi:[1,0]\n\t" \
	"s_nop 0\n\t" \
	"v_pk_add_f32 v[86:87], v[82:83], v[84:85] neg_lo:[0,1] neg_hi:[0,0]\n\t" \
	"s_nop 0\n\t" \
	"v_pk_add_f32 v[120:121], v[120:121], v[86:87]\n\t" \
	"v_pk_mul_f32 v[82:83], v[110:111], v[72:73] op_sel:[0,0] op_sel_hi:[0,1]\n\t" \
	"v_pk_mul_f32 v[84:85], v[110:111], v[72:73] op_sel:[1,1] op_sel_hi:[1,0]\n\t" \
	"s_nop 0\n\t" \
	"v_pk_add_f32 v[86:87], v[82:83], v[84:85] neg_lo:[0,1] neg_hi:[0,0]\n\t" \
	"s_nop 0\n\t" \
	"v_pk_add_f32 v[120:121], v[120:121], v[86:87]\n\t" \
	"v_pk_mul_f32 v[82:83], v[112:113], v[74:75] op_sel:[0,0] op_sel_hi:[0,1]\n\t" \
	"v_pk_mul_f32 v[84:85], v[112:113], v[74:75] op_sel:[1,1] op_sel_hi:[1,0]\n\t" \
	"s_nop 0\n\t" \
	"v_pk_add_f32 v[86:87], v[82:83], v[84:85] neg_lo:[0,1] neg_hi:[0,0]\n\t" \
	"s_nop 0\n\t" \
	"v_pk_add_f32 v[120:121], v[120:121], v[86:87]\n\t" \
	"v_pk_mul_f32 v[82:83], v[114:115], v[76:77] op_sel:[0,0] op_sel_hi:[0,1]\n\t" \
	"v_pk_mul_f32 v[84:85], v[114:115], v[76:77] op_sel:[1,1] op_sel_hi:[1,0]\n\t" \
	"s_nop 0\n\t" \
	"v_pk_add_f32 v[86:87], v[82:83], v[84:85] neg_lo:[0,1] neg_hi:[0,0]\n\t" \
	"s_nop 0\n\t" \
	"v_pk_add_f32 v[120:121], v[120:121], v[86:87]\n\t" \
	"v_pk_mul_f32 v[82:83], v[116:117], v[78:79] op_sel:[0,0] op_sel_hi:[0,1]\n\t" \
	"v_pk_mul_f32 v[84:85], v[116:117], v[78:79] op_sel:[1,1] op_sel_hi:[1,0]\n\t" \
	"s_nop 0\n\t" \
	"v_pk_add_f32 v[86:87], v[82:83], v[84:85] neg_lo:[0,1] neg_hi:[0,0]\n\t" \
	"s_nop 0\n\t" \
	"v_pk_add_f32 v[120:121], v[120:121], v[86:87]\n\t" \
	"v_pk_mul_f32 v[82:83], v[118:119], v[80:81] op_sel:[0,0] op_sel_hi:[0,1]\n\t" \
	"v_pk_mul_f32 v[84:85], v[118:119], v[80:81] op_sel:[1,1] op_sel_hi:[1,0]\n\t" \
	"s_nop 0\n\t" \
	"v_pk_add_f32 v[86:87], v[82:83], v[84:85] neg_lo:[0,1] neg_hi:[0,0]\n\t" \
	"s_nop 0\n\t" \
	"v_pk_add_f32 v[120:121], v[120:121], v[86:87]\n\t" \
	"s_branch .Lnb_corrw_join\n\t" \
	".Lnb_corr_end:\n\t"
#define NB_ASM_DETA \
	"s_mov_b32 %[st], 0\n\t" \
	"s_cmp_lt_i32 %[bidx], 3\n\t" \
	"s_cbranch_scc1 .Lnb_da_end\n\t" \
	"s_sub_u32 s88, %[len], 3\n\t" \
	"s_cmp_gt_i32 %[bidx], s88\n\t" \
	"s_cbranch_scc1 .Lnb_da_end\n\t" \
	"s_lshl3_add_u32 s89, %[bidx], %[czb]\n\t" \
	"s_add_u32 s90, %[len], -1\n\t" \
	"v_mov_b32_e32 v64, s89\n\t" \
	"v_add_u32_e32 v65, s89, %[kr]\n\t" \
	"s_lshl3_add_u32 s90, s90, %[czb]\n\t" \
	"v_add_u32_e32 v66, s89, %[ka]\n\t" \
	"ds_read_b64 v[68:69], v64\n\t" \
	"v_mov_b32_e32 v67, s90\n\t" \
	"v_mov_b64_e32 v[72:73], 0\n\t" \
	"s_bfm_b64 exec, 8, 0\n\t" \
	"ds_read_b64 v[70:71], v65\n\t" \
	"s_mov_b64 exec, 1\n\t" \
	"ds_write_b64 v67, v[72:73]\n\t" \
	"s_mov_b64 exec, -1\n\t" \
	"ds_read_b128 v[76:79], %[l16] offset:16512\n\t" \
	"ds_read_b128 v[80:83], %[l16] offset:17536\n\t" \
	"ds_read_b64 v[88:89], v66 offset:0\n\t" \
	"ds_read_b64 v[90:91], v66 offset:8\n\t" \
	"ds_read_b64 v[92:93], v66 offset:16\n\t" \
	"ds_read_b64 v[94:95], v66 offset:24\n\t" \
	"ds_read_b64 v[96:97], v66 offset:32\n\t" \
	"ds_read_b64 v[98:99], v66 offset:40\n\t" \
	"ds_read_b64 v[100:101], v66 offset:48\n\t" \
	"ds_read_b64 v[102:103], v66 offset:56\n\t" \
	"v_mov_b64_e32 v[84:85], 0\n\t" \
	"v_mov_b64_e32 v[86:87], 0\n\t" \
	"s_add_u32 s91, %[bidx], -1\n\t" \
	"s_sub_u32 s92, %[len], %[bidx]\n\t" \
	"s_min_u32 s91, s91, 4\n\t" \
	"s_waitcnt lgkmcnt(11)\n\t" \
	"v_pk_mul_f32 v[68:69], v[68:69], v[68:69]\n\t" \
	"s_add_u32 s92, s92, -2\n\t" \
	"v_add_f32_e32 v74, v69, v68\n\t" \
	"v_mul_f32_e32 %[km], 0x36c9539c, v74\n\t" \
	"s_bfm_b64 exec, 8, 0\n\t" \
	"v_pk_mul_f32 v[70:71], v[70:71], v[70:71]\n\t" \
	"s_min_u32 s92, s92, 4\n\t" \
	"v_add_f32_e32 v75, v71, v70\n\t" \
	"s_add_u32 s91, s91, s92\n\t" \
	"s_cmp_eq_u32 s91, 8\n\t" \
	"v_add_f32_dpp v75, v75, v75 quad_perm:[1,0,3,2] row_mask:0xf bank_mask:0xf\n\t" \
	"s_cselect_b32 s92, %[k8], %[k7]\n\t" \
	"s_cmp_eq_u32 s91, 6\n\t" \
	"v_add_f32_dpp v75, v75, v75 quad_perm:[2,3,0,1] row_mask:0xf bank_mask:0xf\n\t" \
	"s_cselect_b32 s93, %[k6], %[k5]\n\t" \
	"s_cmp_ge_u32 s91, 7\n\t" \
	"v_add_f32_dpp v75, v75, v75 row_half_mirror row_mask:0xf bank_mask:0xf\n\t" \
	"s_cselect_b32 s92, s92, s93\n\t" \
	"v_mul_f32_e32 v112, s92, v75\n\t" \
	"v_mul_f32_e32 v113, 0x3f7fff37, v112\n\t" \
	"v_fmamk_f32 v114, v112, 0x3f8000c9, %[c0]\n\t" \
	"v_cmp_lt_f32_e32 vcc, v74, v113\n\t" \
	"s_cbranch_vccnz .Lnb_da_wait_end\n\t" \
	"v_cmp_gt_f32_e32 vcc, v74, v114\n\t" \
	"s_mov_b32 %[st], 2\n\t" \
	"s_cbranch_vccz .Lnb_da_wait_end\n\t" \
	"s_mov_b64 exec, -1\n\t" \
	"ds_read_b128 v[104:107], %[l16] offset:18560\n\t" \
	"ds_read_b128 v[108:111], %[l16] offset:19584\n\t" \
	"ds_read_b64 v[112:113], v66 offset:64\n\t" \
	"ds_read_b64 v[114:115], v66 offset:72\n\t" \
	"ds_read_b64 v[116:117], v66 offset:80\n\t" \
	"ds_read_b64 v[118:119], v66 offset:88\n\t" \
	"ds_read_b64 v[120:121], v66 offset:96\n\t" \
	"ds_read_b64 v[122:123], v66 offset:104\n\t" \
	"ds_read_b64 v[124:125], v66 offset:112\n\t" \
	"ds_read_b64 v[126:127], v66 offset:120\n\t" \
	"s_waitcnt lgkmcnt(10)\n\t" \
	"v_pk_fma_f32 v[84:85], v[88:89], v[76:77], v[84:85] op_sel:[0,0,0] op_sel_hi:[1,0,1]\n\t" \
	"v_pk_fma_f32 v[86:87], v[90:91], v[76:77], v[86:87] op_sel:[0,1,0] op_sel_hi:[1,1,1]\n\t" \
	"v_pk_fma_f32 v[84:85], v[92:93], v[78:79], v[84:85] op_sel:[0,0,0] op_sel_hi:[1,0,1]\n\t" \
	"v_pk_fma_f32 v[86:87], v[94:95], v[78:79], v[86:87] op_sel:[0,1,0] op_sel_hi:[1,1,1]\n\t" \
	"v_pk_fma_f32 v[84:85], v[96:97], v[80:81], v[84:85] op_sel:[0,0,0] op_sel_hi:[1,0,1]\n\t" \
	"v_pk_fma_f32 v[86:87], v[98:99], v[80:81], v[86:87] op_sel:[0,1,0] op_sel_hi:[1,1,1]\n\t" \
	"v_pk_fma_f32 v[84:85], v[100:101], v[82:83], v[84:85] op_sel:[0,0,0] op_sel_hi:[1,0,1]\n\t" \
	"v_pk_fma_f32 v[86:87], v[102:103], v[82:83], v[86:87] op_sel:[0,1,0] op_sel_hi:[1,1,1]\n\t" \
	"s_waitcnt lgkmcnt(0)\n\t" \
	"v_pk_fma_f32 v[84:85], v[112:113], v[104:105], v[84:85] op_sel:[0,0,0] op_sel_hi:[1,0,1]\n\t" \
	"v_pk_fma_f32 v[86:87], v[114:115], v[104:105], v[86:87] op_sel:[0,1,0] op_sel_hi:[1,1,1]\n\t" \
	"v_pk_fma_f32 v[84:85], v[116:117], v[106:107], v[84:85] op_sel:[0,0,0] op_sel_hi:[1,0,1]\n\t" \
	"v_pk_fma_f32 v[86:87], v[118:119], v[106:107], v[86:87] op_sel:[0,1,0] op_sel_hi:[1,1,1]\n\t" \
	"v_pk_fma_f32 v[84:85], v[120:121], v[108:109], v[84:85] op_sel:[0,0,0] op_sel_hi:[1,0,1]\n\t" \
	"v_pk_fma_f32 v[86:87], v[122:123], v[108:109], v[86:87] op_sel:[0,1,0] op_sel_hi:[1,1,1]\n\t" \
	"v_pk_fma_f32 v[84:85], v[124:125], v[110:111], v[84:85] op_sel:[0,0,0] op_sel_hi:[1,0,1]\n\t" \
	"v_pk_fma_f32 v[86:87], v[126:127], v[110:111], v[86:87] op_sel:[0,1,0] op_sel_hi:[1,1,1]\n\t" \
	"s_nop 0\n\t" \
	"v_pk_add_f32 v[84:85], v[84:85], v[86:87]\n\t" \
	"s_nop 0\n\t" \
	"v_pk_mul_f32 v[84:85], v[84:85], v[84:85]\n\t" \
	"s_nop 0\n\t" \
	"v_add_f32_e32 v88, v85, v84\n\t" \
	"v_fmamk_f32 v89, v88, 0x36c9539c, %[km]\n\t" \
	"v_sub_f32_e32 v90, v88, v89\n\t" \
	"v_add_f32_e32 v91, v88, v89\n\t" \
	"s_lshl_b32 s94, %[bidx], 9\n\t" \
	"v_mov_b32_dpp v90, v90 quad_perm:[1,0,3,2] row_mask:0xf bank_mask:0xf\n\t" \
	"v_cmp_lt_f32_e64 s[88:89], v91, v90\n\t" \
	"s_mov_b32 %[st], 1\n\t" \
	"s_lshr_b64 s[90:91], s[88:89], 1\n\t" \
	"s_or_b64 s[90:91], s[90:91], s[88:89]\n\t" \
	"s_mov_b32 s96, 0x55555555\n\t" \
	"s_mov_b32 s97, 0x15555555\n\t" \
	"s_and_b64 s[92:93], s[90:91], s[96:97]\n\t" \
	"s_cmp_eq_u64 s[92:93], s[96:97]\n\t" \
	"s_cbranch_scc0 .Lnb_da_careful\n\t" \
	"s_mov_b32 s95, 0\n\t" \
	"s_lshl1_add_u32 s96, s95, 0\n\t" \
	"s_bitcmp1_b64 s[88:89], s96\n\t" \
	"s_addc_u32 s95, s95, s95\n\t" \
	"s_lshl1_add_u32 s96, s95, 2\n\t" \
	"s_bitcmp1_b64 s[88:89], s96\n\t" \
	"s_addc_u32 s95, s95, s95\n\t" \
	"s_lshl1_add_u32 s96, s95, 6\n\t" \
	"s_bitcmp1_b64 s[88:89], s96\n\t" \
	"s_addc_u32 s95, s95, s95\n\t" \
	"s_lshl1_add_u32 s96, s95, 14\n\t" \
	"s_bitcmp1_b64 s[88:89], s96\n\t" \
	"s_addc_u32 s95, s95, s95\n\t" \
	"s_lshl1_add_u32 s96, s95, 30\n\t" \
	"s_bitcmp1_b64 s[88:89], s96\n\t" \
	"s_addc_u32 s95, s95, s95\n\t" \
	".Lnb_da_walked:\n\t" \
	"s_lshl_b32 s95, s95, 5\n\t" \
	"s_add_u32 s94, s94, s95\n\t" \
	"s_add_u32 %[e], s94, -1008\n\t" \
	"s_branch .Lnb_da_end\n\t" \
	".Lnb_da_careful:\n\t" \
	"s_mov_b32 s95, 0\n\t" \
	"s_lshl1_add_u32 s96, s95, 0\n\t" \
	"s_bitcmp0_b64 s[90:91], s96\n\t" \
	"s_cbranch_scc1 .Lnb_da_unsure\n\t" \
	"s_bitcmp1_b64 s[88:89], s96\n\t" \
	"s_addc_u32 s95, s95, s95\n\t" \
	"s_lshl1_add_u32 s96, s95, 2\n\t" \
	"s_bitcmp0_b64 s[90:91], s96\n\t" \
	"s_cbranch_scc1 .Lnb_da_unsure\n\t" \
	"s_bitcmp1_b64 s[88:89], s96\n\t" \
	"s_addc_u32 s95, s95, s95\n\t" \
	"s_lshl1_add_u32 s96, s95, 6\n\t" \
	"s_bitcmp0_b64 s[90:91], s96\n\t" \
	"s_cbranch_scc1 .Lnb_da_unsure\n\t" \
	"s_bitcmp1_b64 s[88:89], s96\n\t" \
	"s_addc_u32 s95, s95, s95\n\t" \
	"s_lshl1_add_u32 s96, s95, 14\n\t" \
	"s_bitcmp0_b64 s[90:91], s96\n\t" \
	"s_cbranch_scc1 .Lnb_da_unsure\n\t" \
	"s_bitcmp1_b64 s[88:89], s96\n\t" \
	"s_addc_u32 s95, s95, s95\n\t" \
	"s_lshl1_add_u32 s96, s95, 30\n\t" \
	"s_bitcmp0_b64 s[90:91], s96\n\t" \
	"s_cbranch_scc1 .Lnb_da_unsure\n\t" \
	"s_bitcmp1_b64 s[88:89], s96\n\t" \
	"s_addc_u32 s95, s95, s95\n\t" \
	"s_branch .Lnb_da_walked\n\t" \
	".Lnb_da_unsure:\n\t" \
	"s_mov_b32 %[st], 3\n\t" \
	"s_branch .Lnb_da_end\n\t" \
	".Lnb_da_wait_end:\n\t" \
	"s_mov_b64 exec, -1\n\t" \
	"s_waitcnt lgkmcnt(0)\n\t" \
	".Lnb_da_end:\n\t"
#define NB_ASM_DETB \
	"v_mov_b64_e32 v[64:65], 0\n\t" \
	"v_mov_b64_e32 v[66:67], 0\n\t" \
	"v_add_u32_e32 v68, %[e], %[kb]\n\t" \
	"s_add_u32 s88, %[czb], -56\n\t" \
	"s_mov_b32 exec_lo, 0x3fffffff\n\t" \
	"s_mov_b32 exec_hi, 0xffff\n\t" \
	"v_ashrrev_i32_e32 v69, 9, v68\n\t" \
	"v_and_b32_e32 v70, 0x1ff, v68\n\t" \
	"v_lshl_add_u32 v69, v69, 3, s88\n\t" \
	"v_bfe_u32 v71, v70, 4, 5\n\t" \
	"v_sub_u32_e32 v72, 0x200, v70\n\t" \
	"v_xor_b32_e32 v71, v71, v70\n\t" \
	"v_bfe_u32 v73, v72, 4, 5\n\t" \
	"v_lshlrev_b32_e32 v71, 2, v71\n\t" \
	"v_xor_b32_e32 v72, v73, v72\n\t" \
	"v_lshlrev_b32_e32 v72, 2, v72\n\t" \
	"ds_read_b64 v[80:81], v69 offset:0\n\t" \
	"ds_read_b32 v96, v71 offset:14336\n\t" \
	"ds_read_b64 v[82:83], v69 offset:8\n\t" \
	"ds_read_b32 v97, v71 offset:12288\n\t" \
	"ds_read_b64 v[84:85], v69 offset:16\n\t" \
	"ds_read_b32 v98, v71 offset:10240\n\t" \
	"ds_read_b64 v[86:87], v69 offset:24\n\t" \
	"ds_read_b32 v99, v71 offset:8192\n\t" \
	"ds_read_b64 v[88:89], v69 offset:32\n\t" \
	"ds_read_b32 v100, v71 offset:6144\n\t" \
	"ds_read_b64 v[90:91], v69 offset:40\n\t" \
	"ds_read_b32 v101, v71 offset:4096\n\t" \
	"ds_read_b64 v[92:93], v69 offset:48\n\t" \
	"ds_read_b32 v102, v71 offset:2048\n\t" \
	"ds_read_b64 v[94:95], v69 offset:56\n\t" \
	"ds_read_b32 v103, v71 offset:0\n\t" \
	"s_waitcnt lgkmcnt(12)\n\t" \
	"v_pk_fma_f32 v[64:65], v[80:81], v[96:97], v[64:65] op_sel:[0,0,0] op_sel_hi:[1,0,1]\n\t" \
	"v_pk_fma_f32 v[66:67], v[82:83], v[96:97], v[66:67] op_sel:[0,1,0] op_sel_hi:[1,1,1]\n\t" \
	"ds_read_b64 v[104:105], v69 offset:64\n\t" \
	"ds_read_b32 v120, v72 offset:0\n\t" \
	"ds_read_b64 v[106:107], v69 offset:72\n\t" \
	"ds_read_b32 v121, v72 offset:2048\n\t" \
	"s_waitcnt lgkmcnt(12)\n\t" \
	"v_pk_fma_f32 v[64:65], v[84:85], v[98:99], v[64:65] op_sel:[0,0,0] op_sel_hi:[1,0,1]\n\t" \
	"v_pk_fma_f32 v[66:67], v[86:87], v[98:99], v[66:67] op_sel:[0,1,0] op_sel_hi:[1,1,1]\n\t" \
	"ds_read_b64 v[108:109], v69 offset:80\n\t" \
	"ds_read_b32 v122, v72 offset:4096\n\t" \
	"ds_read_b64 v[110:111], v69 offset:88\n\t" \
	"ds_read_b32 v123, v72 offset:6144\n\t" \
	"s_waitcnt lgkmcnt(12)\n\t" \
	"v_pk_fma_f32 v[64:65], v[88:89], v[100:101], v[64:65] op_sel:[0,0,0] op_sel_hi:[1,0,1]\n\t" \
	"v_pk_fma_f32 v[66:67], v[90:91], v[100:101], v[66:67] op_sel:[0,1,0] op_sel_hi:[1,1,1]\n\t" \
	"ds_read_b64 v[112:113], v69 offset:96\n\t" \
	"ds_read_b32 v124, v72 offset:8192\n\t" \
	"ds_read_b64 v[114:115], v69 offset:104\n\t" \
	"ds_read_b32 v125, v72 offset:10240\n\t" \
	"s_waitcnt lgkmcnt(12)\n\t" \
	"v_pk_fma_f32 v[64:65], v[92:93], v[102:103], v[64:65] op_sel:[0,0,0] op_sel_hi:[1,0,1]\n\t" \
	"v_pk_fma_f32 v[66:67], v[94:95], v[102:103], v[66:67] op_sel:[0,1,0] op_sel_hi:[1,1,1]\n\t" \
	"ds_read_b64 v[116:117], v69 offset:112\n\t" \
	"ds_read_b32 v126, v72 offset:12288\n\t" \
	"ds_read_b64 v[118:119], v69 offset:120\n\t" \
	"ds_read_b32 v127, v72 offset:14336\n\t" \
	"s_waitcnt lgkmcnt(12)\n\t" \
	"v_pk_fma_f32 v[64:65], v[104:105], v[120:121], v[64:65] op_sel:[0,0,0] op_sel_hi:[1,0,1]\n\t" \
	"v_pk_fma_f32 v[66:67], v[106:107], v[120:121], v[66:67] op_sel:[0,1,0] op_sel_hi:[1,1,1]\n\t" \
	"s_waitcnt lgkmcnt(8)\n\t" \
	"v_pk_fma_f32 v[64:65], v[108:109], v[122:123], v[64:65] op_sel:[0,0,0] op_sel_hi:[1,0,1]\n\t" \
	"v_pk_fma_f32 v[66:67], v[110:111], v[122:123], v[66:67] op_sel:[0,1,0] op_sel_hi:[1,1,1]\n\t" \
	"s_waitcnt lgkmcnt(4)\n\t" \
	"v_pk_fma_f32 v[64:65], v[112:113], v[124:125], v[64:65] op_sel:[0,0,0] op_sel_hi:[1,0,1]\n\t" \
	"v_pk_fma_f32 v[66:67], v[114:115], v[124:125], v[66:67] op_sel:[0,1,0] op_sel_hi:[1,1,1]\n\t" \
	"s_waitcnt lgkmcnt(0)\n\t" \
	"v_pk_fma_f32 v[64:65], v[116:117], v[126:127], v[64:65] op_sel:[0,0,0] op_sel_hi:[1,0,1]\n\t" \
	"v_pk_fma_f32 v[66:67], v[118:119], v[126:127], v[66:67] op_sel:[0,1,0] op_sel_hi:[1,1,1]\n\t" \
	"s_mov_b64 exec, -1\n\t" \
	"v_pk_add_f32 v[74:75], v[64:65], v[66:67]\n\t" \
	"s_add_u32 s92, %[e], 497\n\t" \
	"v_pk_mul_f32 v[76:77], v[74:75], v[74:75]\n\t" \
	"s_mov_b32 %[st], 1\n\t" \
	"v_add_f32_e32 v78, v77, v76\n\t" \
	"v_fmamk_f32 v79, v78, 0x36c9539c, %[km]\n\t" \
	"v_sub_f32_e32 v96, v78, v79\n\t" \
	"v_add_f32_e32 v97, v78, v79\n\t" \
	"s_nop 0\n\t" \
	"v_mov_b32_dpp v96, v96 quad_perm:[1,0,3,2] row_mask:0xf bank_mask:0xf\n\t" \
	"v_cmp_lt_f32_e64 s[88:89], v97, v96\n\t" \
	"s_lshr_b32 s90, s88, 1\n\t" \
	"s_or_b32 s90, s90, s88\n\t" \
	"s_and_b32 s91, s90, 0x15555555\n\t" \
	"s_cmp_eq_u32 s91, 0x15555555\n\t" \
	"s_cbranch_scc0 .Lnb_db_careful\n\t" \
	"s_mov_b32 s94, 0\n\t" \
	"s_lshl1_add_u32 s95, s94, 0\n\t" \
	"s_bitcmp1_b32 s88, s95\n\t" \
	"s_addc_u32 s94, s94, s94\n\t" \
	"s_lshl1_add_u32 s95, s94, 2\n\t" \
	"s_bitcmp1_b32 s88, s95\n\t" \
	"s_addc_u32 s94, s94, s94\n\t" \
	"s_lshl1_add_u32 s95, s94, 6\n\t" \
	"s_bitcmp1_b32 s88, s95\n\t" \
	"s_addc_u32 s94, s94, s94\n\t" \
	"s_lshl1_add_u32 s95, s94, 14\n\t" \
	"s_bitcmp1_b32 s88, s95\n\t" \
	"s_addc_u32 s94, s94, s94\n\t" \
	".Lnb_db_walked:\n\t" \
	"s_add_u32 s93, s94, 32\n\t" \
	"s_lshl1_add_u32 %[toa], s94, s92\n\t" \
	"v_readlane_b32 %[xr], v74, s93\n\t" \
	"v_readlane_b32 %[xi], v75, s93\n\t" \
	"s_branch .Lnb_db_end\n\t" \
	".Lnb_db_careful:\n\t" \
	"s_mov_b32 s94, 0\n\t" \
	"s_lshl1_add_u32 s95, s94, 0\n\t" \
	"s_bitcmp0_b32 s90, s95\n\t" \
	"s_cbranch_scc1 .Lnb_db_unsure\n\t" \
	"s_bitcmp1_b32 s88, s95\n\t" \
	"s_addc_u32 s94, s94, s94\n\t" \
	"s_lshl1_add_u32 s95, s94, 2\n\t" \
	"s_bitcmp0_b32 s90, s95\n\t" \
	"s_cbranch_scc1 .Lnb_db_unsure\n\t" \
	"s_bitcmp1_b32 s88, s95\n\t" \
	"s_addc_u32 s94, s94, s94\n\t" \
	"s_lshl1_add_u32 s95, s94, 6\n\t" \
	"s_bitcmp0_b32 s90, s95\n\t" \
	"s_cbranch_scc1 .Lnb_db_unsure\n\t" \
	"s_bitcmp1_b32 s88, s95\n\t" \
	"s_addc_u32 s94, s94, s94\n\t" \
	"s_lshl1_add_u32 s95, s94, 14\n\t" \
	"s_bitcmp0_b32 s90, s95\n\t" \
	"s_cbranch_scc1 .Lnb_db_unsure\n\t" \
	"s_bitcmp1_b32 s88, s95\n\t" \
	"s_addc_u32 s94, s94, s94\n\t" \
	"s_branch .Lnb_db_walked\n\t" \
	".Lnb_db_unsure:\n\t" \
	"s_mov_b32 %[st], 3\n\t" \
	".Lnb_db_end:\n\t"
#define NB_ASM_TAIL \
	"v_mov_b32_e32 v65, %[hdrb]\n\t" \
	"ds_read_b128 v[68:71], v65\n\t" \
	"s_sub_u32 s88, %[t5], %[toa]\n\t" \
	"s_add_u32 s87, s88, 5120\n\t" \
	"s_mov_b32 %[ok], 0\n\t" \
	"s_and_b32 s91, s87, 127\n\t" \
	"s_lshr_b32 s92, s91, 1\n\t" \
	"s_cmp_ge_u32 s91, 2\n\t" \
	"s_cselect_b32 s92, s92, 64\n\t" \
	"s_mul_i32 s93, s92, 768\n\t" \
	"s_add_u32 s94, %[e8lo], s93\n\t" \
	"s_addc_u32 s95, %[e8hi], 0\n\t" \
	"s_abs_i32 s96, %[toa]\n\t" \
	"s_add_u32 s96, s96, 256\n\t" \
	"global_load_dwordx4 v[120:123], %[l16], s[94:95]\n\t" \
	"s_lshr_b32 s96, s96, 9\n\t" \
	"s_sub_u32 s97, 0, s96\n\t" \
	"s_cmp_lt_i32 %[toa], 0\n\t" \
	"s_cselect_b32 s96, s97, s96\n\t" \
	"s_lshl_b32 s96, s96, 3\n\t" \
	"v_add_u32_e32 v64, s96, %[vd]\n\t" \
	"s_bfm_b64 exec, 16, 0\n\t" \
	"ds_read_b64 v[66:67], v64\n\t" \
	"s_mov_b64 exec, -1\n\t" \
	"s_waitcnt lgkmcnt(1)\n\t" \
	"v_mul_f32_e32 v82, %[xr], v70\n\t" \
	"v_mul_f32_e32 v83, %[xr], v71\n\t" \
	"v_mul_f32_e32 v84, %[xi], v71\n\t" \
	"v_mul_f32_e32 v85, %[xi], v70\n\t" \
	"v_sub_f32_e32 v86, v82, v84\n\t" \
	"v_add_f32_e32 v87, v83, v85\n\t" \
	"v_mul_f32_e32 v90, v86, v86\n\t" \
	"v_mul_f32_e32 v89, v87, v87\n\t" \
	"v_add_f32_e32 v89, v89, v90\n\t" \
	"v_rcp_f32_e32 v89, v89\n\t" \
	"s_mov_b32 s88, 0xaaaaaaaa\n\t" \
	"s_mov_b32 s89, 0xaaaaaaaa\n\t" \
	"v_mul_f32_e32 v91, v86, v89\n\t" \
	"v_mul_f32_e64 v92, -v87, v89\n\t" \
	"v_cndmask_b32_e64 v119, v91, v92, s[88:89]\n\t" \
	"s_mov_b32 s88, 0xcccccccc\n\t" \
	"s_mov_b32 s89, 0xcccccccc\n\t" \
	"v_cndmask_b32_e64 v119, v119, -v119, s[88:89]\n\t" \
	"s_bfm_b64 exec, 16, 0\n\t" \
	"s_waitcnt lgkmcnt(0)\n\t" \
	"v_pk_mul_f32 v[66:67], v[66:67], v[66:67]\n\t" \
	"s_ashr_i32 s88, s87, 7\n\t" \
	"v_add_f32_e32 v81, v67, v66\n\t" \
	"s_and_b32 s89, s87, 127\n\t" \
	"s_lshr_b32 s90, s89, 1\n\t" \
	"v_add_f32_dpp v81, v81, v81 quad_perm:[1,0,3,2] row_mask:0xf bank_mask:0xf\n\t" \
	"s_cmp_ge_u32 s89, 2\n\t" \
	"s_cselect_b32 s90, s90, 64\n\t" \
	"v_add_f32_dpp v81, v81, v81 quad_perm:[2,3,0,1] row_mask:0xf bank_mask:0xf\n\t" \
	"s_sub_u32 s91, -18, s88\n\t" \
	"s_and_b32 s92, s91, 3\n\t" \
	"v_add_f32_dpp v81, v81, v81 row_half_mirror row_mask:0xf bank_mask:0xf\n\t" \
	"s_ashr_i32 s93, s91, 2\n\t" \
	"s_mul_i32 s94, s92, 180\n\t" \
	"v_add_f32_dpp v81, v81, v81 row_mirror row_mask:0xf bank_mask:0xf\n\t" \
	"s_add_u32 s94, s94, s93\n\t" \
	"s_lshl3_add_u32 s94, s94, %[pb]\n\t" \
	"v_mul_f32_e32 v81, 0x3d800000, v81\n\t" \
	"s_mul_i32 s95, s90, 144\n\t" \
	"s_add_u32 s95, s95, %[cb]\n\t" \
	"v_readlane_b32 %[ssum], v81, 0\n\t" \
	"s_mov_b64 exec, -1\n\t" \
	"s_sub_u32 s96, 0, s88\n\t" \
	"s_cmp_gt_u32 s96, 36\n\t" \
	"s_cbranch_scc1 .Lnb_tl_wait_end\n\t" \
	"s_mov_b32 %[ok], 1\n\t" \
	"v_add_u32_e32 v112, s94, %[kic]\n\t" \
	"s_add_u32 s96, s92, 1\n\t" \
	"s_lshr_b32 s96, s96, 2\n\t" \
	"s_mul_i32 s96, s96, -5752\n\t" \
	"s_add_u32 s96, s96, 1440\n\t" \
	"v_add_u32_e32 v113, s96, v112\n\t" \
	"s_add_u32 s96, s92, 2\n\t" \
	"s_lshr_b32 s96, s96, 2\n\t" \
	"s_mul_i32 s96, s96, -5752\n\t" \
	"s_add_u32 s96, s96, 2880\n\t" \
	"v_add_u32_e32 v114, s96, v112\n\t" \
	"s_add_u32 s96, s92, 3\n\t" \
	"s_lshr_b32 s96, s96, 2\n\t" \
	"s_mul_i32 s96, s96, -5752\n\t" \
	"s_add_u32 s96, s96, 4320\n\t" \
	"v_add_u32_e32 v115, s96, v112\n\t" \
	"ds_read_b64 v[72:73], v112 offset:96\n\t" \
	"ds_read_b64 v[74:75], v113 offset:96\n\t" \
	"ds_read_b64 v[76:77], v114 offset:96\n\t" \
	"ds_read_b64 v[78:79], v115 offset:96\n\t" \
	"ds_read_b64 v[80:81], v112 offset:104\n\t" \
	"ds_read_b64 v[82:83], v113 offset:104\n\t" \
	"ds_read_b64 v[84:85], v114 offset:104\n\t" \
	"ds_read_b64 v[86:87], v115 offset:104\n\t" \
	"ds_read_b64 v[88:89], v112 offset:112\n\t" \
	"ds_read_b64 v[90:91], v113 offset:112\n\t" \
	"ds_read_b64 v[92:93], v114 offset:112\n\t" \
	"ds_read_b64 v[94:95], v115 offset:112\n\t" \
	"v_add_u32_e32 v116, %[db], %[l16]\n\t" \
	"v_cmp_lt_i32_e32 vcc, -1, %[ktp]\n\t" \
	"v_add_u32_e32 v117, %[db], %[ktp]\n\t" \
	"v_mov_b32_e32 v118, s95\n\t" \
	"v_mov_b64_e32 v[64:65], 0\n\t" \
	"v_mov_b64_e32 v[66:67], 0\n\t" \
	"v_mov_b64_e32 v[68:69], 0\n\t" \
	"v_cndmask_b32_e32 v117, v118, v117, vcc\n\t" \
	"s_waitcnt vmcnt(0)\n\t" \
	"ds_write_b128 v116, v[120:123]\n\t" \
	"ds_read_b128 v[96:99], v117 offset:0\n\t" \
	"ds_read_b128 v[100:103], v117 offset:16\n\t" \
	"ds_read_b128 v[104:107], v117 offset:32\n\t" \
	"ds_read_b128 v[108:111], v117 offset:48\n\t" \
	"ds_read_b128 v[124:127], v117 offset:64\n\t" \
	"s_waitcnt lgkmcnt(4)\n\t" \
	"ds_read_b128 v[120:123], v117 offset:80\n\t" \
	"v_pk_fma_f32 v[64:65], v[72:73], v[96:97], v[64:65] op_sel:[0,0,0] op_sel_hi:[1,0,1]\n\t" \
	"v_pk_fma_f32 v[66:67], v[80:81], v[96:97], v[66:67] op_sel:[0,0,0] op_sel_hi:[1,0,1]\n\t" \
	"v_pk_fma_f32 v[68:69], v[88:89], v[96:97], v[68:69] op_sel:[0,0,0] op_sel_hi:[1,0,1]\n\t" \
	"v_pk_fma_f32 v[64:65], v[74:75], v[96:97], v[64:65] op_sel:[0,1,0] op_sel_hi:[1,1,1]\n\t" \
	"v_pk_fma_f32 v[66:67], v[82:83], v[96:97], v[66:67] op_sel:[0,1,0] op_sel_hi:[1,1,1]\n\t" \
	"v_pk_fma_f32 v[68:69], v[90:91], v[96:97], v[68:69] op_sel:[0,1,0] op_sel_hi:[1,1,1]\n\t" \
	"v_pk_fma_f32 v[64:65], v[76:77], v[98:99], v[64:65] op_sel:[0,0,0] op_sel_hi:[1,0,1]\n\t" \
	"v_pk_fma_f32 v[66:67], v[84:85], v[98:99], v[66:67] op_sel:[0,0,0] op_sel_hi:[1,0,1]\n\t" \
	"v_pk_fma_f32 v[68:69], v[92:93], v[98:99], v[68:69] op_sel:[0,0,0] op_sel_hi:[1,0,1]\n\t" \
	"v_pk_fma_f32 v[64:65], v[78:79], v[98:99], v[64:65] op_sel:[0,1,0] op_sel_hi:[1,1,1]\n\t" \
	"v_pk_fma_f32 v[66:67], v[86:87], v[98:99], v[66:67] op_sel:[0,1,0] op_sel_hi:[1,1,1]\n\t" \
	"v_pk_fma_f32 v[68:69], v[94:95], v[98:99], v[68:69] op_sel:[0,1,0] op_sel_hi:[1,1,1]\n\t" \
	"s_waitcnt lgkmcnt(4)\n\t" \
	"v_pk_fma_f32 v[64:65], v[80:81], v[100:101], v[64:65] op_sel:[0,0,0] op_sel_hi:[1,0,1]\n\t" \
	"v_pk_fma_f32 v[66:67], v[88:89], v[100:101], v[66:67] op_sel:[0,0,0] op_sel_hi:[1,0,1]\n\t" \
	"v_mov_b32_dpp v68, v68 wave_shr:1 row_mask:0xf bank_mask:0xf bound_ctrl:0\n\t" \
	"v_mov_b32_dpp v69, v69 wave_shr:1 row_mask:0xf bank_mask:0xf bound_ctrl:0\n\t" \
	"v_pk_fma_f32 v[64:65], v[82:83], v[100:101], v[64:65] op_sel:[0,1,0] op_sel_hi:[1,1,1]\n\t" \
	"v_pk_fma_f32 v[66:67], v[90:91], v[100:101], v[66:67] op_sel:[0,1,0] op_sel_hi:[1,1,1]\n\t" \
	"v_pk_fma_f32 v[68:69], v[72:73], v[100:101], v[68:69] op_sel:[0,0,0] op_sel_hi:[1,0,1]\n\t" \
	"v_pk_fma_f32 v[64:65], v[84:85], v[102:103], v[64:65] op_sel:[0,0,0] op_sel_hi:[1,0,1]\n\t" \
	"v_pk_fma_f32 v[66:67], v[92:93], v[102:103], v[66:67] op_sel:[0,0,0] op_sel_hi:[1,0,1]\n\t" \
	"v_pk_fma_f32 v[68:69], v[74:75], v[100:101], v[68:69] op_sel:[0,1,0] op_sel_hi:[1,1,1]\n\t" \
	"v_pk_fma_f32 v[64:65], v[86:87], v[102:103], v[64:65] op_sel:[0,1,0] op_sel_hi:[1,1,1]\n\t" \
	"v_pk_fma_f32 v[66:67], v[94:95], v[102:103], v[66:67] op_sel:[0,1,0] op_sel_hi:[1,1,1]\n\t" \
	"v_pk_fma_f32 v[68:69], v[76:77], v[102:103], v[68:69] op_sel:[0,0,0] op_sel_hi:[1,0,1]\n\t" \
	"s_waitcnt lgkmcnt(3)\n\t" \
	"v_pk_fma_f32 v[64:65], v[88:89], v[104:105], v[64:65] op_sel:[0,0,0] op_sel_hi:[1,0,1]\n\t" \
	"s_bfm_b64 exec, 52, 0\n\t" \
	"v_mov_b32_dpp v66, v66 wave_shr:1 row_mask:0xf bank_mask:0xf bound_ctrl:0\n\t" \
	"v_mov_b32_dpp v67, v67 wave_shr:1 row_mask:0xf bank_mask:0xf bound_ctrl:0\n\t" \
	"s_mov_b64 exec, -1\n\t" \
	"v_pk_fma_f32 v[68:69], v[78:79], v[102:103], v[68:69] op_sel:[0,1,0] op_sel_hi:[1,1,1]\n\t" \
	"v_pk_fma_f32 v[64:65], v[90:91], v[104:105], v[64:65] op_sel:[0,1,0] op_sel_hi:[1,1,1]\n\t" \
	"v_pk_fma_f32 v[66:67], v[72:73], v[104:105], v[66:67] op_sel:[0,0,0] op_sel_hi:[1,0,1]\n\t" \
	"v_pk_fma_f32 v[68:69], v[80:81], v[104:105], v[68:69] op_sel:[0,0,0] op_sel_hi:[1,0,1]\n\t" \
	"v_pk_fma_f32 v[64:65], v[92:93], v[106:107], v[64:65] op_sel:[0,0,0] op_sel_hi:[1,0,1]\n\t" \
	"v_pk_fma_f32 v[66:67], v[74:75], v[104:105], v[66:67] op_sel:[0,1,0] op_sel_hi:[1,1,1]\n\t" \
	"v_pk_fma_f32 v[68:69], v[82:83], v[104:105], v[68:69] op_sel:[0,1,0] op_sel_hi:[1,1,1]\n\t" \
	"v_pk_fma_f32 v[64:65], v[94:95], v[106:107], v[64:65] op_sel:[0,1,0] op_sel_hi:[1,1,1]\n\t" \
	"v_pk_fma_f32 v[66:67], v[76:77], v[106:107], v[66:67] op_sel:[0,0,0] op_sel_hi:[1,0,1]\n\t" \
	"v_pk_fma_f32 v[68:69], v[84:85], v[106:107], v[68:69] op_sel:[0,0,0] op_sel_hi:[1,0,1]\n\t" \
	"v_mov_b32_dpp v64, v64 wave_shr:1 row_mask:0xf bank_mask:0xf bound_ctrl:0\n\t" \
	"v_mov_b32_dpp v65, v65 wave_shr:1 row_mask:0xf bank_mask:0xf bound_ctrl:0\n\t" \
	"v_pk_fma_f32 v[66:67], v[78:79], v[106:107], v[66:67] op_sel:[0,1,0] op_sel_hi:[1,1,1]\n\t" \
	"v_pk_fma_f32 v[68:69], v[86:87], v[106:107], v[68:69] op_sel:[0,1,0] op_sel_hi:[1,1,1]\n\t" \
	"s_waitcnt lgkmcnt(2)\n\t" \
	"v_pk_fma_f32 v[64:65], v[72:73], v[108:109], v[64:65] op_sel:[0,0,0] op_sel_hi:[1,0,1]\n\t" \
	"v_pk_fma_f32 v[66:67], v[80:81], v[108:109], v[66:67] op_sel:[0,0,0] op_sel_hi:[1,0,1]\n\t" \
	"v_pk_fma_f32 v[68:69], v[88:89], v[108:109], v[68:69] op_sel:[0,0,0] op_sel_hi:[1,0,1]\n\t" \
	"v_pk_fma_f32 v[64:65], v[74:75], v[108:109], v[64:65] op_sel:[0,1,0] op_sel_hi:[1,1,1]\n\t" \
	"v_pk_fma_f32 v[66:67], v[82:83], v[108:109], v[66:67] op_sel:[0,1,0] op_sel_hi:[1,1,1]\n\t" \
	"v_pk_fma_f32 v[68:69], v[90:91], v[108:109], v[68:69] op_sel:[0,1,0] op_sel_hi:[1,1,1]\n\t" \
	"v_pk_fma_f32 v[64:65], v[76:77], v[110:111], v[64:65] op_sel:[0,0,0] op_sel_hi:[1,0,1]\n\t" \
	"v_pk_fma_f32 v[66:67], v[84:85], v[110:111], v[66:67] op_sel:[0,0,0] op_sel_hi:[1,0,1]\n\t" \
	"v_pk_fma_f32 v[68:69], v[92:93], v[110:111], v[68:69] op_sel:[0,0,0] op_sel_hi:[1,0,1]\n\t" \
	"v_pk_fma_f32 v[64:65], v[78:79], v[110:111], v[64:65] op_sel:[0,1,0] op_sel_hi:[1,1,1]\n\t" \
	"v_pk_fma_f32 v[66:67], v[86:87], v[110:111], v[66:67] op_sel:[0,1,0] op_sel_hi:[1,1,1]\n\t" \
	"v_pk_fma_f32 v[68:69], v[94:95], v[110:111], v[68:69] op_sel:[0,1,0] op_sel_hi:[1,1,1]\n\t" \
	"s_waitcnt lgkmcnt(1)\n\t" \
	"v_pk_fma_f32 v[64:65], v[80:81], v[124:125], v[64:65] op_sel:[0,0,0] op_sel_hi:[1,0,1]\n\t" \
	"v_pk_fma_f32 v[66:67], v[88:89], v[124:125], v[66:67] op_sel:[0,0,0] op_sel_hi:[1,0,1]\n\t" \
	"v_mov_b32_dpp v68, v68 wave_shr:1 row_mask:0xf bank_mask:0xf bound_ctrl:0\n\t" \
	"v_mov_b32_dpp v69, v69 wave_shr:1 row_mask:0xf bank_mask:0xf bound_ctrl:0\n\t" \
	"v_pk_fma_f32 v[64:65], v[82:83], v[124:125], v[64:65] op_sel:[0,1,0] op_sel_hi:[1,1,1]\n\t" \
	"v_pk_fma_f32 v[66:67], v[90:91], v[124:125], v[66:67] op_sel:[0,1,0] op_sel_hi:[1,1,1]\n\t" \
	"v_pk_fma_f32 v[68:69], v[72:73], v[124:125], v[68:69] op_sel:[0,0,0] op_sel_hi:[1,0,1]\n\t" \
	"v_pk_fma_f32 v[64:65], v[84:85], v[126:127], v[64:65] op_sel:[0,0,0] op_sel_hi:[1,0,1]\n\t" \
	"v_pk_fma_f32 v[66:67], v[92:93], v[126:127], v[66:67] op_sel:[0,0,0] op_sel_hi:[1,0,1]\n\t" \
	"v_pk_fma_f32 v[68:69], v[74:75], v[124:125], v[68:69] op_sel:[0,1,0] op_sel_hi:[1,1,1]\n\t" \
	"v_pk_fma_f32 v[64:65], v[86:87], v[126:127], v[64:65] op_sel:[0,1,0] op_sel_hi:[1,1,1]\n\t" \
	"v_pk_fma_f32 v[66:67], v[94:95], v[126:127], v[66:67] op_sel:[0,1,0] op_sel_hi:[1,1,1]\n\t" \
	"v_pk_fma_f32 v[68:69], v[76:77], v[126:127], v[68:69] op_sel:[0,0,0] op_sel_hi:[1,0,1]\n\t" \
	"s_waitcnt lgkmcnt(0)\n\t" \
	"v_pk_fma_f32 v[64:65], v[88:89], v[120:121], v[64:65] op_sel:[0,0,0] op_sel_hi:[1,0,1]\n\t" \
	"s_bfm_b64 exec, 52, 0\n\t" \
	"v_mov_b32_dpp v66, v66 wave_shr:1 row_mask:0xf bank_mask:0xf bound_ctrl:0\n\t" \
	"v_mov_b32_dpp v67, v67 wave_shr:1 row_mask:0xf bank_mask:0xf bound_ctrl:0\n\t" \
	"s_mov_b64 exec, -1\n\t" \
	"v_pk_fma_f32 v[68:69], v[78:79], v[126:127], v[68:69] op_sel:[0,1,0] op_sel_hi:[1,1,1]\n\t" \
	"v_pk_fma_f32 v[64:65], v[90:91], v[120:121], v[64:65] op_sel:[0,1,0] op_sel_hi:[1,1,1]\n\t" \
	"v_pk_fma_f32 v[66:67], v[72:73], v[120:121], v[66:67] op_sel:[0,0,0] op_sel_hi:[1,0,1]\n\t" \
	"v_pk_fma_f32 v[68:69], v[80:81], v[120:121], v[68:69] op_sel:[0,0,0] op_sel_hi:[1,0,1]\n\t" \
	"v_pk_fma_f32 v[64:65], v[92:93], v[122:123], v[64:65] op_sel:[0,0,0] op_sel_hi:[1,0,1]\n\t" \
	"v_pk_fma_f32 v[66:67], v[74:75], v[120:121], v[66:67] op_sel:[0,1,0] op_sel_hi:[1,1,1]\n\t" \
	"v_pk_fma_f32 v[68:69], v[82:83], v[120:121], v[68:69] op_sel:[0,1,0] op_sel_hi:[1,1,1]\n\t" \
	"v_pk_fma_f32 v[64:65], v[94:95], v[122:123], v[64:65] op_sel:[0,1,0] op_sel_hi:[1,1,1]\n\t" \
	"v_pk_fma_f32 v[66:67], v[76:77], v[122:123], v[66:67] op_sel:[0,0,0] op_sel_hi:[1,0,1]\n\t" \
	"v_pk_fma_f32 v[68:69], v[84:85], v[122:123], v[68:69] op_sel:[0,0,0] op_sel_hi:[1,0,1]\n\t" \
	"v_mov_b32_dpp v64, v64 wave_shr:1 row_mask:0xf bank_mask:0xf bound_ctrl:0\n\t" \
	"v_mov_b32_dpp v65, v65 wave_shr:1 row_mask:0xf bank_mask:0xf bound_ctrl:0\n\t" \
	"v_pk_fma_f32 v[66:67], v[78:79], v[122:123], v[66:67] op_sel:[0,1,0] op_sel_hi:[1,1,1]\n\t" \
	"v_pk_fma_f32 v[68:69], v[86:87], v[122:123], v[68:69] op_sel:[0,1,0] op_sel_hi:[1,1,1]\n\t" \
	"s_mov_b32 exec_lo, 0\n\t" \
	"s_mov_b32 exec_hi, 0xfff00000\n\t" \
	"v_pk_add_f32 v[64:65], v[64:65], v[66:67]\n\t" \
	"s_mov_b64 exec, -1\n\t" \
	"v_mul_f32_dpp %[d1], v119, v66 quad_perm:[3,2,1,0] row_mask:0xf bank_mask:0xf\n\t" \
	"v_mul_f32_dpp %[d2], v119, v68 quad_perm:[0,3,2,1] row_mask:0xf bank_mask:0xf\n\t" \
	"v_mul_f32_dpp %[d0], v119, v64 quad_perm:[2,1,0,3] row_mask:0xf bank_mask:0xf\n\t" \
	"v_fmac_f32_dpp %[d1], v119, v67 quad_perm:[2,1,0,3] row_mask:0xf bank_mask:0xf\n\t" \
	"v_fmac_f32_dpp %[d2], v119, v69 quad_perm:[3,2,1,0] row_mask:0xf bank_mask:0xf\n\t" \
	"v_fmac_f32_dpp %[d0], v119, v65 quad_perm:[1,0,3,2] row_mask:0xf bank_mask:0xf\n\t" \
	"s_branch .Lnb_tl_end\n\t" \
	".Lnb_tl_wait_end:\n\t" \
	"s_waitcnt vmcnt(0)\n\t" \
	".Lnb_tl_end:\n\t"
#define NB_ASM_FIRG \
	"s_ashr_i32 s88, %[nk], 7\n\t" \
	"s_and_b32 s89, %[nk], 127\n\t" \
	"s_lshr_b32 s90, s89, 1\n\t" \
	"s_cmp_ge_u32 s89, 2\n\t" \
	"s_cselect_b32 s90, s90, 64\n\t" \
	"s_sub_u32 s91, -18, s88\n\t" \
	"s_and_b32 s92, s91, 3\n\t" \
	"s_ashr_i32 s93, s91, 2\n\t" \
	"s_mul_i32 s94, s92, 180\n\t" \
	"s_add_u32 s94, s94, s93\n\t" \
	"s_lshl3_add_u32 s94, s94, %[pb]\n\t" \
	"s_mul_i32 s95, s90, 144\n\t" \
	"s_add_u32 s95, s95, %[cb]\n\t" \
	"v_add_u32_e32 v112, s94, %[kic]\n\t" \
	"s_add_u32 s96, s92, 1\n\t" \
	"s_lshr_b32 s96, s96, 2\n\t" \
	"s_mul_i32 s96, s96, -5752\n\t" \
	"s_add_u32 s96, s96, 1440\n\t" \
	"v_add_u32_e32 v113, s96, v112\n\t" \
	"s_add_u32 s96, s92, 2\n\t" \
	"s_lshr_b32 s96, s96, 2\n\t" \
	"s_mul_i32 s96, s96, -5752\n\t" \
	"s_add_u32 s96, s96, 2880\n\t" \
	"v_add_u32_e32 v114, s96, v112\n\t" \
	"s_add_u32 s96, s92, 3\n\t" \
	"s_lshr_b32 s96, s96, 2\n\t" \
	"s_mul_i32 s96, s96, -5752\n\t" \
	"s_add_u32 s96, s96, 4320\n\t" \
	"v_add_u32_e32 v115, s96, v112\n\t" \
	"v_mov_b64_e32 %[a0], 0\n\t" \
	"v_mov_b64_e32 %[a1], 0\n\t" \
	"v_mov_b64_e32 %[a2], 0\n\t" \
	"v_mov_b32_e32 v117, s95\n\t" \
	"s_bfm_b64 exec, 52, 0\n\t" \
	"ds_read_b64 v[72:73], v112 offset:96\n\t" \
	"ds_read_b64 v[74:75], v113 offset:96\n\t" \
	"ds_read_b64 v[76:77], v114 offset:96\n\t" \
	"ds_read_b64 v[78:79], v115 offset:96\n\t" \
	"ds_read_b64 v[80:81], v112 offset:104\n\t" \
	"ds_read_b64 v[82:83], v113 offset:104\n\t" \
	"ds_read_b64 v[84:85], v114 offset:104\n\t" \
	"ds_read_b64 v[86:87], v115 offset:104\n\t" \
	"ds_read_b64 v[88:89], v112 offset:112\n\t" \
	"ds_read_b64 v[90:91], v113 offset:112\n\t" \
	"ds_read_b64 v[92:93], v114 offset:112\n\t" \
	"ds_read_b64 v[94:95], v115 offset:112\n\t" \
	"ds_read_b128 v[104:107], v117\n\t" \
	"ds_read_b128 v[108:111], v117 offset:16\n\t" \
	"ds_read_b64 v[96:97], v112 offset:120\n\t" \
	"ds_read_b64 v[98:99], v113 offset:120\n\t" \
	"ds_read_b64 v[100:101], v114 offset:120\n\t" \
	"ds_read_b64 v[102:103], v115 offset:120\n\t" \
	"s_waitcnt lgkmcnt(5)\n\t" \
	"v_pk_fma_f32 %[a0], v[72:73], v[104:105], %[a0] op_sel:[0,0,0] op_sel_hi:[1,0,1]\n\t" \
	"v_pk_fma_f32 %[a1], v[80:81], v[104:105], %[a1] op_sel:[0,0,0] op_sel_hi:[1,0,1]\n\t" \
	"v_pk_fma_f32 %[a2], v[88:89], v[104:105], %[a2] op_sel:[0,0,0] op_sel_hi:[1,0,1]\n\t" \
	"v_pk_fma_f32 %[a0], v[74:75], v[104:105], %[a0] op_sel:[0,1,0] op_sel_hi:[1,1,1]\n\t" \
	"v_pk_fma_f32 %[a1], v[82:83], v[104:105], %[a1] op_sel:[0,1,0] op_sel_hi:[1,1,1]\n\t" \
	"v_pk_fma_f32 %[a2], v[90:91], v[104:105], %[a2] op_sel:[0,1,0] op_sel_hi:[1,1,1]\n\t" \
	"v_pk_fma_f32 %[a0], v[76:77], v[106:107], %[a0] op_sel:[0,0,0] op_sel_hi:[1,0,1]\n\t" \
	"v_pk_fma_f32 %[a1], v[84:85], v[106:107], %[a1] op_sel:[0,0,0] op_sel_hi:[1,0,1]\n\t" \
	"v_pk_fma_f32 %[a2], v[92:93], v[106:107], %[a2] op_sel:[0,0,0] op_sel_hi:[1,0,1]\n\t" \
	"v_pk_fma_f32 %[a0], v[78:79], v[106:107], %[a0] op_sel:[0,1,0] op_sel_hi:[1,1,1]\n\t" \
	"v_pk_fma_f32 %[a1], v[86:87], v[106:107], %[a1] op_sel:[0,1,0] op_sel_hi:[1,1,1]\n\t" \
	"v_pk_fma_f32 %[a2], v[94:95], v[106:107], %[a2] op_sel:[0,1,0] op_sel_hi:[1,1,1]\n\t" \
	"ds_read_b128 v[104:107], v117 offset:32\n\t" \
	"ds_read_b64 v[72:73], v112 offset:128\n\t" \
	"ds_read_b64 v[74:75], v113 offset:128\n\t" \
	"ds_read_b64 v[76:77], v114 offset:128\n\t" \
	"ds_read_b64 v[78:79], v115 offset:128\n\t" \
	"s_waitcnt lgkmcnt(5)\n\t" \
	"v_pk_fma_f32 %[a0], v[80:81], v[108:109], %[a0] op_sel:[0,0,0] op_sel_hi:[1,0,1]\n\t" \
	"v_pk_fma_f32 %[a1], v[88:89], v[108:109], %[a1] op_sel:[0,0,0] op_sel_hi:[1,0,1]\n\t" \
	"v_pk_fma_f32 %[a2], v[96:97], v[108:109], %[a2] op_sel:[0,0,0] op_sel_hi:[1,0,1]\n\t" \
	"v_pk_fma_f32 %[a0], v[82:83], v[108:109], %[a0] op_sel:[0,1,0] op_sel_hi:[1,1,1]\n\t" \
	"v_pk_fma_f32 %[a1], v[90:91], v[108:109], %[a1] op_sel:[0,1,0] op_sel_hi:[1,1,1]\n\t" \
	"v_pk_fma_f32 %[a2], v[98:99], v[108:109], %[a2] op_sel:[0,1,0] op_sel_hi:[1,1,1]\n\t" \
// ... 101 lines not shown
```

Measured before the change: 1093.

## Merge peak-detect rounds A and B and reuse round A's LDS samples in round B

Fuses the two inline-asm peak detection stages into one block so the correlation samples loaded for the coarse round stay in registers and are reused by the fine round, instead of round B recomputing addresses and reloading 16 samples from LDS. The sinc-weight table is rotated per lane, and per-lane shifts are handled with EXEC-masked FMAs. Round B's weight addresses are precomputed as XOR-swizzled offsets in a lookup table. Loads are widened to ds_read2_b64. This adds masking complexity, a branch on the sample parity, and constexpr checks that must stay in step with the generator script.

Result: no change. 1102, median of 6 (+0.8%).

```diff
diff --git a/osmo_trx_amd/csrc/trx_kernel_nb.hip b/osmo_trx_amd/csrc/trx_kernel_nb.hip
--- a/osmo_trx_amd/csrc/trx_kernel_nb.hip
+++ b/osmo_trx_amd/csrc/trx_kernel_nb.hip
@@ -20,6 +20,29 @@
 
 typedef float v3f __attribute__((ext_vector_type(3)));
 typedef int v4i __attribute__((ext_vector_type(4)));
+
+constexpr int nb_node_offset(int n, int inc0)
+{
+	int L = 0;
+	while ((2 << L) <= n + 1)
+		L++;
+	const int p = n + 1 - (1 << L);
+	return ((4 * p * inc0) >> L) - (2 * inc0 - ((2 * inc0) >> L));
+}
+constexpr bool nb_det_final(int l) { return l >= 32 && l < 48; }
+constexpr int nb_det_window(int l) { return nb_det_final(l) ? -8 : (l & 1) ? -7 : -9; }
+constexpr int nb_det_shift_a(int l) { return -8 + ((nb_node_offset(l >> 1, 256) + ((l & 1) ? 1024 : 0)) >> 9) - nb_det_window(l); }
+constexpr int nb_det_g(int l) { return l < 30 ? 16 + nb_node_offset(l >> 1, 8) : nb_det_final(l) ? 2 * (l & 15) + 1 : 16; }
+constexpr unsigned long long nb_det_shift_mask(int k)
+{
+	unsigned long long m = 0;
+	for (int l = 0; l < WAVE; l++)
+		m |= (nb_det_shift_a(l) == k) ? 1ull << l : 0ull;
+	return m;
+}
+static_assert(nb_det_shift_mask(-1) == NB_ASM_DET_SHIFT_M1 && nb_det_shift_mask(0) == NB_ASM_DET_SHIFT_0 &&
+	      nb_det_shift_mask(1) == NB_ASM_DET_SHIFT_1 && nb_det_shift_mask(2) == NB_ASM_DET_SHIFT_2,
+	      "tools/gen_nb_asm.py: round A's EXEC masks and the staging of wa4 below assume the same lane geometry");
 
 template <typename T>
 __device__ __forceinline__ unsigned lds_addr(const T *p)
@@ -45,7 +68,6 @@
 
 	float *const sincv = reinterpret_cast<float *>(smem);
 	float *const wa4f = sincv + TRX_SINCV_LDS;
-	const float4 *const wa4 = reinterpret_cast<const float4 *>(wa4f);
 	float *const comp = wa4f + 16 * WAVE;
 	float *const gdec = comp + NB_COMP_ROWS * 36;
 	float *const lhdr = gdec + 16;
@@ -65,7 +87,8 @@
 		const int l = i & (WAVE - 1), u = i >> 6;
 		const PeakConst pcl = peak_const(l);
 		const int q = (u < 8) ? pcl.loA + 512 * (7 - u) : pcl.hiA + 512 * (u - 8);
-		wa4f[((u >> 2) * WAVE + l) * 4 + (u & 3)] = (q < TRX_SINCV_LEN) ? tab->sincv[q] : 0.0f;
+		const int k = (u + nb_det_shift_a(l) + 1) & 15;
+		wa4f[((k >> 2) * WAVE + l) * 4 + (k & 3)] = (q < TRX_SINCV_LEN) ? tab->sincv[q] : 0.0f;
 	}
 	for (int i = threadIdx.x; i < NB_COMP_ROWS * 36; i += blockDim.x) {
 		const int f = i / 36, j = i % 36;
@@ -85,9 +108,10 @@
 		pkcl[2 * WAVE + threadIdx.x] = pc0.hiA;
 		pkcl[3 * WAVE + threadIdx.x] = pc0.offB;
 		pkcl[4 * WAVE + threadIdx.x] = pc0.ratio_off;
+		const int g = nb_det_g(threadIdx.x), gc = 32 - g;
 		lcn[0 * WAVE + threadIdx.x] = pc0.ratio_off * 8;
-		lcn[1 * WAVE + threadIdx.x] = (pc0.flA - 8) * 8;
-		lcn[2 * WAVE + threadIdx.x] = pc0.offB;
+		lcn[1 * WAVE + threadIdx.x] = nb_det_window(threadIdx.x) * 8;
+		lcn[2 * WAVE + threadIdx.x] = (4 * (g ^ (g >> 4))) | ((4 * (gc ^ (gc >> 4))) << 16);
 		const int l = threadIdx.x, e = (l - 52) / 3, t = (l - 52) % 3;
 		const bool sp = l >= 52;
 		lcn[3 * WAVE + l] = 8 * (sp ? (t == 0 ? e : t == 1 ? e + 3 : e - 3) : 4 + 3 * (l < 49 ? l : 49));
@@ -412,22 +436,14 @@
 				int hit = 0;
 				int toa512 = 0;
 				if (m_bits != 0) {
-					int st, e512;
+					int st, e512, xr_bits, xi_bits;
 					float km;
-					asm volatile(NB_ASM_DETA
-						     : [st] "=&s"(st), [e] "=&s"(e512), [km] "=&v"(km)
-						     : [bidx] "s"(bidx), [len] "s"(len), [czb] "s"(lds_addr(cz)), [kr] "v"(kr), [ka] "v"(ka), [l16] "v"(16 * lane),
-						       [k5] "s"(gk5), [k6] "s"(gk6), [k7] "s"(gk7), [k8] "s"(gk8), [c0] "v"(gc0)
+					asm volatile(NB_ASM_DET
+						     : [st] "=&s"(st), [e] "=&s"(e512), [km] "=&v"(km), [toa] "=&s"(toa512), [xr] "=&s"(xr_bits), [xi] "=&s"(xi_bits)
+						     : [bidx] "s"(bidx), [len] "s"(len), [czb] "s"(lds_addr(cz)), [kr] "v"(kr), [ka] "v"(ka), [kb] "v"(kb),
+						       [l16] "v"(16 * lane), [k5] "s"(gk5), [k6] "s"(gk6), [k7] "s"(gk7), [k8] "s"(gk8), [c0] "v"(gc0)
 						     : NB_ASM_CLOBBERS);
 					DIAG_MARK(5);
-					int xr_bits = 0, xi_bits = 0;
-					if (st == 1) {
-						asm volatile(NB_ASM_DETB
-							     : [st] "=&s"(st), [toa] "=&s"(toa512), [xr] "=&s"(xr_bits), [xi] "=&s"(xi_bits)
-							     : [e] "s"(e512), [kb] "v"(kb), [czb] "s"(lds_addr(cz)), [km] "v"(km)
-							     : NB_ASM_CLOBBERS);
-						DIAG_MARK(6);
-					}
 					if (st == 3) {
 						if (lane == 0)
 							atomicAdd(&g_trx_fast_stats[0], 1ull);
@@ -435,7 +451,7 @@
 						pkc.flA = pkcl[0 * WAVE + lane]; pkc.loA = pkcl[1 * WAVE + lane]; pkc.hiA = pkcl[2 * WAVE + lane];
 						pkc.offB = pkcl[3 * WAVE + lane]; pkc.ratio_off = pkcl[4 * WAVE + lane];
 						c32 xcorr;
-						peak_detect_spec(cz, bidx, sincv, pkc, lane, &toa512, &xcorr, wa4);
+						peak_detect_spec(cz, bidx, sincv, pkc, lane, &toa512, &xcorr, nullptr);
 						toa512 = uni(toa512);
 						xr_bits = uni(__float_as_int(xcorr.x));
 						xi_bits = uni(__float_as_int(xcorr.y));
diff --git a/osmo_trx_amd/csrc/trx_nb_asm.inc b/osmo_trx_amd/csrc/trx_nb_asm.inc
--- a/osmo_trx_amd/csrc/trx_nb_asm.inc
+++ b/osmo_trx_amd/csrc/trx_nb_asm.inc
@@ -3,6 +3,10 @@
 #define NB_ASM_DEC_MAX_NACT 60
 #define NB_ASM_CORR_LANE0 19
 #define NB_ASM_CORR_MAX_LEN 45
+#define NB_ASM_DET_SHIFT_M1 0x0000155500000000ull
+#define NB_ASM_DET_SHIFT_0 0xc0004000c03fc3ccull
+#define NB_ASM_DET_SHIFT_1 0x3fff2aaa3fc03c33ull
+#define NB_ASM_DET_SHIFT_2 0x0000800000000000ull
 #define NB_ASM_CLOBBERS "v64", "v65", "v66", "v67", "v68", "v69", "v70", "v71", "v72", "v73", "v74", "v75", "v76", "v77", "v78", "v79", "v80", "v81", "v82", "v83", "v84", "v85", "v86", "v87", "v88", "v89", "v90", "v91", "v92", "v93", "v94", "v95", "v96", "v97", "v98", "v99", "v100", "v101", "v102", "v103", "v104", "v105", "v106", "v107", "v108", "v109", "v110", "v111", "v112", "v113", "v114", "v115", "v116", "v117", "v118", "v119", "v120", "v121", "v122", "v123", "v124", "v125", "v126", "v127", "s87", "s88", "s89", "s90", "s91", "s92", "s93", "s94", "s95", "s96", "s97", "s98", "s99", "vcc", "scc", "memory"
 #define NB_ASM_DEC \
 	"s_cmp_gt_u32 %[nact], 60\n\t" \
@@ -1103,13 +1107,13 @@
 	"v_pk_add_f32 v[120:121], v[120:121], v[86:87]\n\t" \
 	"s_branch .Lnb_corrw_join\n\t" \
 	".Lnb_corr_end:\n\t"
-#define NB_ASM_DETA \
+#define NB_ASM_DET \
 	"s_mov_b32 %[st], 0\n\t" \
 	"s_cmp_lt_i32 %[bidx], 3\n\t" \
-	"s_cbranch_scc1 .Lnb_da_end\n\t" \
+	"s_cbranch_scc1 .Lnb_db_end\n\t" \
 	"s_sub_u32 s88, %[len], 3\n\t" \
 	"s_cmp_gt_i32 %[bidx], s88\n\t" \
-	"s_cbranch_scc1 .Lnb_da_end\n\t" \
+	"s_cbranch_scc1 .Lnb_db_end\n\t" \
 	"s_lshl3_add_u32 s89, %[bidx], %[czb]\n\t" \
 	"s_add_u32 s90, %[len], -1\n\t" \
 	"v_mov_b32_e32 v64, s89\n\t" \
@@ -1119,27 +1123,27 @@
 	"ds_read_b64 v[68:69], v64\n\t" \
 	"v_mov_b32_e32 v67, s90\n\t" \
 	"v_mov_b64_e32 v[72:73], 0\n\t" \
+	"s_add_u32 s94, s89, -72\n\t" \
+	"v_and_b32_e32 v124, 16, %[l16]\n\t" \
 	"s_bfm_b64 exec, 8, 0\n\t" \
 	"ds_read_b64 v[70:71], v65\n\t" \
 	"s_mov_b64 exec, 1\n\t" \
 	"ds_write_b64 v67, v[72:73]\n\t" \
 	"s_mov_b64 exec, -1\n\t" \
+	"v_mad_u32_u24 v124, v124, 9, s94\n\t" \
 	"ds_read_b128 v[76:79], %[l16] offset:16512\n\t" \
 	"ds_read_b128 v[80:83], %[l16] offset:17536\n\t" \
-	"ds_read_b64 v[88:89], v66 offset:0\n\t" \
-	"ds_read_b64 v[90:91], v66 offset:8\n\t" \
-	"ds_read_b64 v[92:93], v66 offset:16\n\t" \
-	"ds_read_b64 v[94:95], v66 offset:24\n\t" \
-	"ds_read_b64 v[96:97], v66 offset:32\n\t" \
-	"ds_read_b64 v[98:99], v66 offset:40\n\t" \
-	"ds_read_b64 v[100:101], v66 offset:48\n\t" \
-	"ds_read_b64 v[102:103], v66 offset:56\n\t" \
+	"ds_read_b64 v[122:123], v124\n\t" \
+	"ds_read2_b64 v[88:91], v66 offset0:0 offset1:1\n\t" \
+	"ds_read2_b64 v[92:95], v66 offset0:2 offset1:3\n\t" \
+	"ds_read2_b64 v[96:99], v66 offset0:4 offset1:5\n\t" \
+	"ds_read2_b64 v[100:103], v66 offset0:6 offset1:7\n\t" \
 	"v_mov_b64_e32 v[84:85], 0\n\t" \
 	"v_mov_b64_e32 v[86:87], 0\n\t" \
 	"s_add_u32 s91, %[bidx], -1\n\t" \
 	"s_sub_u32 s92, %[len], %[bidx]\n\t" \
 	"s_min_u32 s91, s91, 4\n\t" \
-	"s_waitcnt lgkmcnt(11)\n\t" \
+	"s_waitcnt lgkmcnt(8)\n\t" \
 	"v_pk_mul_f32 v[68:69], v[68:69], v[68:69]\n\t" \
 	"s_add_u32 s92, s92, -2\n\t" \
 	"v_add_f32_e32 v74, v69, v68\n\t" \
@@ -1167,46 +1171,60 @@
 	"s_mov_b32 %[st], 2\n\t" \
 	"s_cbranch_vccz .Lnb_da_wait_end\n\t" \
 	"s_mov_b64 exec, -1\n\t" \
-	"ds_read_b128 v[104:107], %[l16] offset:18560\n\t" \
-	"ds_read_b128 v[108:111], %[l16] offset:19584\n\t" \
-	"ds_read_b64 v[112:113], v66 offset:64\n\t" \
-	"ds_read_b64 v[114:115], v66 offset:72\n\t" \
-	"ds_read_b64 v[116:117], v66 offset:80\n\t" \
-	"ds_read_b64 v[118:119], v66 offset:88\n\t" \
-	"ds_read_b64 v[120:121], v66 offset:96\n\t" \
-	"ds_read_b64 v[122:123], v66 offset:104\n\t" \
-	"ds_read_b64 v[124:125], v66 offset:112\n\t" \
-	"ds_read_b64 v[126:127], v66 offset:120\n\t" \
-	"s_waitcnt lgkmcnt(10)\n\t" \
-	"v_pk_fma_f32 v[84:85], v[88:89], v[76:77], v[84:85] op_sel:[0,0,0] op_sel_hi:[1,0,1]\n\t" \
-	"v_pk_fma_f32 v[86:87], v[90:91], v[76:77], v[86:87] op_sel:[0,1,0] op_sel_hi:[1,1,1]\n\t" \
-	"v_pk_fma_f32 v[84:85], v[92:93], v[78:79], v[84:85] op_sel:[0,0,0] op_sel_hi:[1,0,1]\n\t" \
-	"v_pk_fma_f32 v[86:87], v[94:95], v[78:79], v[86:87] op_sel:[0,1,0] op_sel_hi:[1,1,1]\n\t" \
-	"v_pk_fma_f32 v[84:85], v[96:97], v[80:81], v[84:85] op_sel:[0,0,0] op_sel_hi:[1,0,1]\n\t" \
-	"v_pk_fma_f32 v[86:87], v[98:99], v[80:81], v[86:87] op_sel:[0,1,0] op_sel_hi:[1,1,1]\n\t" \
-	"v_pk_fma_f32 v[84:85], v[100:101], v[82:83], v[84:85] op_sel:[0,0,0] op_sel_hi:[1,0,1]\n\t" \
-	"v_pk_fma_f32 v[86:87], v[102:103], v[82:83], v[86:87] op_sel:[0,1,0] op_sel_hi:[1,1,1]\n\t" \
-	"s_waitcnt lgkmcnt(0)\n\t" \
-	"v_pk_fma_f32 v[84:85], v[112:113], v[104:105], v[84:85] op_sel:[0,0,0] op_sel_hi:[1,0,1]\n\t" \
-	"v_pk_fma_f32 v[86:87], v[114:115], v[104:105], v[86:87] op_sel:[0,1,0] op_sel_hi:[1,1,1]\n\t" \
-	"v_pk_fma_f32 v[84:85], v[116:117], v[106:107], v[84:85] op_sel:[0,0,0] op_sel_hi:[1,0,1]\n\t" \
-	"v_pk_fma_f32 v[86:87], v[118:119], v[106:107], v[86:87] op_sel:[0,1,0] op_sel_hi:[1,1,1]\n\t" \
-	"v_pk_fma_f32 v[84:85], v[120:121], v[108:109], v[84:85] op_sel:[0,0,0] op_sel_hi:[1,0,1]\n\t" \
-	"v_pk_fma_f32 v[86:87], v[122:123], v[108:109], v[86:87] op_sel:[0,1,0] op_sel_hi:[1,1,1]\n\t" \
-	"v_pk_fma_f32 v[84:85], v[124:125], v[110:111], v[84:85] op_sel:[0,0,0] op_sel_hi:[1,0,1]\n\t" \
-	"v_pk_fma_f32 v[86:87], v[126:127], v[110:111], v[86:87] op_sel:[0,1,0] op_sel_hi:[1,1,1]\n\t" \
-	"s_nop 0\n\t" \
+	"ds_read_b128 v[68:71], %[l16] offset:18560\n\t" \
+	"ds_read_b128 v[72:75], %[l16] offset:19584\n\t" \
+	"ds_read2_b64 v[104:107], v66 offset0:8 offset1:9\n\t" \
+	"ds_read2_b64 v[108:111], v66 offset0:10 offset1:11\n\t" \
+	"ds_read2_b64 v[112:115], v66 offset0:12 offset1:13\n\t" \
+	"ds_read2_b64 v[116:119], v66 offset0:14 offset1:15\n\t" \
+	"ds_read_b64 v[120:121], v66 offset:128\n\t" \
+	"s_waitcnt lgkmcnt(7)\n\t" \
+	"s_mov_b32 exec_lo, 0x00000000\n\t" \
+	"s_mov_b32 exec_hi, 0x00001555\n\t" \
+	"v_pk_fma_f32 v[86:87], v[122:123], v[76:77], v[86:87] op_sel:[0,0,0] op_sel_hi:[1,0,1]\n\t" \
+	"s_mov_b32 exec_lo, 0xc03fc3cc\n\t" \
+	"s_mov_b32 exec_hi, 0xc0005555\n\t" \
+	"v_pk_fma_f32 v[84:85], v[88:89], v[76:77], v[84:85] op_sel:[0,1,0] op_sel_hi:[1,1,1]\n\t" \
+	"s_mov_b32 exec_lo, 0xffffffff\n\t" \
+	"s_mov_b32 exec_hi, 0xffff7fff\n\t" \
+	"v_pk_fma_f32 v[86:87], v[90:91], v[78:79], v[86:87] op_sel:[0,0,0] op_sel_hi:[1,0,1]\n\t" \
+	"s_mov_b64 exec, -1\n\t" \
+	"v_pk_fma_f32 v[84:85], v[92:93], v[78:79], v[84:85] op_sel:[0,1,0] op_sel_hi:[1,1,1]\n\t" \
+	"v_pk_fma_f32 v[86:87], v[94:95], v[80:81], v[86:87] op_sel:[0,0,0] op_sel_hi:[1,0,1]\n\t" \
+	"v_pk_fma_f32 v[84:85], v[96:97], v[80:81], v[84:85] op_sel:[0,1,0] op_sel_hi:[1,1,1]\n\t" \
+	"v_pk_fma_f32 v[86:87], v[98:99], v[82:83], v[86:87] op_sel:[0,0,0] op_sel_hi:[1,0,1]\n\t" \
+	"v_pk_fma_f32 v[84:85], v[100:101], v[82:83], v[84:85] op_sel:[0,1,0] op_sel_hi:[1,1,1]\n\t" \
+	"s_waitcnt lgkmcnt(3)\n\t" \
+	"v_pk_fma_f32 v[86:87], v[102:103], v[68:69], v[86:87] op_sel:[0,0,0] op_sel_hi:[1,0,1]\n\t" \
+	"v_pk_fma_f32 v[84:85], v[104:105], v[68:69], v[84:85] op_sel:[0,1,0] op_sel_hi:[1,1,1]\n\t" \
+	"v_pk_fma_f32 v[86:87], v[106:107], v[70:71], v[86:87] op_sel:[0,0,0] op_sel_hi:[1,0,1]\n\t" \
+	"v_pk_fma_f32 v[84:85], v[108:109], v[70:71], v[84:85] op_sel:[0,1,0] op_sel_hi:[1,1,1]\n\t" \
+	"v_pk_fma_f32 v[86:87], v[110:111], v[72:73], v[86:87] op_sel:[0,0,0] op_sel_hi:[1,0,1]\n\t" \
+	"s_waitcnt lgkmcnt(0)\n\t" \
+	"v_pk_fma_f32 v[84:85], v[112:113], v[72:73], v[84:85] op_sel:[0,1,0] op_sel_hi:[1,1,1]\n\t" \
+	"v_pk_fma_f32 v[86:87], v[114:115], v[74:75], v[86:87] op_sel:[0,0,0] op_sel_hi:[1,0,1]\n\t" \
+	"v_pk_fma_f32 v[84:85], v[116:117], v[74:75], v[84:85] op_sel:[0,1,0] op_sel_hi:[1,1,1]\n\t" \
+	"s_mov_b32 exec_lo, 0xffffffff\n\t" \
+	"s_mov_b32 exec_hi, 0xffffeaaa\n\t" \
+	"v_pk_fma_f32 v[86:87], v[118:119], v[76:77], v[86:87] op_sel:[0,0,0] op_sel_hi:[1,0,1]\n\t" \
+	"s_mov_b32 exec_lo, 0x3fc03c33\n\t" \
+	"s_mov_b32 exec_hi, 0x3fffaaaa\n\t" \
+	"v_pk_fma_f32 v[84:85], v[120:121], v[76:77], v[84:85] op_sel:[0,1,0] op_sel_hi:[1,1,1]\n\t" \
+	"s_mov_b32 exec_lo, 0x00000000\n\t" \
+	"s_mov_b32 exec_hi, 0x00008000\n\t" \
+	"v_pk_fma_f32 v[86:87], v[122:123], v[78:79], v[86:87] op_sel:[0,0,0] op_sel_hi:[1,0,1]\n\t" \
+	"s_mov_b64 exec, -1\n\t" \
 	"v_pk_add_f32 v[84:85], v[84:85], v[86:87]\n\t" \
 	"s_nop 0\n\t" \
 	"v_pk_mul_f32 v[84:85], v[84:85], v[84:85]\n\t" \
 	"s_nop 0\n\t" \
-	"v_add_f32_e32 v88, v85, v84\n\t" \
-	"v_fmamk_f32 v89, v88, 0x36c9539c, %[km]\n\t" \
-	"v_sub_f32_e32 v90, v88, v89\n\t" \
-	"v_add_f32_e32 v91, v88, v89\n\t" \
+	"v_add_f32_e32 v64, v85, v84\n\t" \
+	"v_fmamk_f32 v65, v64, 0x36c9539c, %[km]\n\t" \
+	"v_sub_f32_e32 v66, v64, v65\n\t" \
+	"v_add_f32_e32 v67, v64, v65\n\t" \
 	"s_lshl_b32 s94, %[bidx], 9\n\t" \
-	"v_mov_b32_dpp v90, v90 quad_perm:[1,0,3,2] row_mask:0xf bank_mask:0xf\n\t" \
-	"v_cmp_lt_f32_e64 s[88:89], v91, v90\n\t" \
+	"v_mov_b32_dpp v66, v66 quad_perm:[1,0,3,2] row_mask:0xf bank_mask:0xf\n\t" \
+	"v_cmp_lt_f32_e64 s[88:89], v67, v66\n\t" \
 	"s_mov_b32 %[st], 1\n\t" \
 	"s_lshr_b64 s[90:91], s[88:89], 1\n\t" \
 	"s_or_b64 s[90:91], s[90:91], s[88:89]\n\t" \
@@ -1232,118 +1250,91 @@
 	"s_bitcmp1_b64 s[88:89], s96\n\t" \
 	"s_addc_u32 s95, s95, s95\n\t" \
 	".Lnb_da_walked:\n\t" \
-	"s_lshl_b32 s95, s95, 5\n\t" \
-	"s_add_u32 s94, s94, s95\n\t" \
+	"s_lshl_b32 s96, s95, 5\n\t" \
+	"s_and_b32 s97, s95, 15\n\t" \
+	"s_add_u32 s94, s94, s96\n\t" \
+	"s_mul_i32 s98, s97, 136\n\t" \
+	"s_sub_u32 s97, 15, s97\n\t" \
 	"s_add_u32 %[e], s94, -1008\n\t" \
-	"s_branch .Lnb_da_end\n\t" \
-	".Lnb_da_careful:\n\t" \
-	"s_mov_b32 s95, 0\n\t" \
-	"s_lshl1_add_u32 s96, s95, 0\n\t" \
-	"s_bitcmp0_b64 s[90:91], s96\n\t" \
-	"s_cbranch_scc1 .Lnb_da_unsure\n\t" \
-	"s_bitcmp1_b64 s[88:89], s96\n\t" \
-	"s_addc_u32 s95, s95, s95\n\t" \
-	"s_lshl1_add_u32 s96, s95, 2\n\t" \
-	"s_bitcmp0_b64 s[90:91], s96\n\t" \
-	"s_cbranch_scc1 .Lnb_da_unsure\n\t" \
-	"s_bitcmp1_b64 s[88:89], s96\n\t" \
-	"s_addc_u32 s95, s95, s95\n\t" \
-	"s_lshl1_add_u32 s96, s95, 6\n\t" \
-	"s_bitcmp0_b64 s[90:91], s96\n\t" \
-	"s_cbranch_scc1 .Lnb_da_unsure\n\t" \
-	"s_bitcmp1_b64 s[88:89], s96\n\t" \
-	"s_addc_u32 s95, s95, s95\n\t" \
-	"s_lshl1_add_u32 s96, s95, 14\n\t" \
-	"s_bitcmp0_b64 s[90:91], s96\n\t" \
-	"s_cbranch_scc1 .Lnb_da_unsure\n\t" \
-	"s_bitcmp1_b64 s[88:89], s96\n\t" \
-	"s_addc_u32 s95, s95, s95\n\t" \
-	"s_lshl1_add_u32 s96, s95, 30\n\t" \
-	"s_bitcmp0_b64 s[90:91], s96\n\t" \
-	"s_cbranch_scc1 .Lnb_da_unsure\n\t" \
-	"s_bitcmp1_b64 s[88:89], s96\n\t" \
-	"s_addc_u32 s95, s95, s95\n\t" \
-	"s_branch .Lnb_da_walked\n\t" \
-	".Lnb_da_unsure:\n\t" \
-	"s_mov_b32 %[st], 3\n\t" \
-	"s_branch .Lnb_da_end\n\t" \
-	".Lnb_da_wait_end:\n\t" \
-	"s_mov_b64 exec, -1\n\t" \
-	"s_waitcnt lgkmcnt(0)\n\t" \
-	".Lnb_da_end:\n\t"
-#define NB_ASM_DETB \
+	"s_mul_i32 s97, s97, 136\n\t" \
+	"s_lshl_b32 s97, s97, 16\n\t" \
+	"s_or_b32 s98, s98, s97\n\t" \
 	"v_mov_b64_e32 v[64:65], 0\n\t" \
 	"v_mov_b64_e32 v[66:67], 0\n\t" \
-	"v_add_u32_e32 v68, %[e], %[kb]\n\t" \
-	"s_add_u32 s88, %[czb], -56\n\t" \
+	"v_xor_b32_e32 v70, s98, %[kb]\n\t" \
 	"s_mov_b32 exec_lo, 0x3fffffff\n\t" \
 	"s_mov_b32 exec_hi, 0xffff\n\t" \
-	"v_ashrrev_i32_e32 v69, 9, v68\n\t" \
-	"v_and_b32_e32 v70, 0x1ff, v68\n\t" \
-	"v_lshl_add_u32 v69, v69, 3, s88\n\t" \
-	"v_bfe_u32 v71, v70, 4, 5\n\t" \
-	"v_sub_u32_e32 v72, 0x200, v70\n\t" \
-	"v_xor_b32_e32 v71, v71, v70\n\t" \
-	"v_bfe_u32 v73, v72, 4, 5\n\t" \
-	"v_lshlrev_b32_e32 v71, 2, v71\n\t" \
-	"v_xor_b32_e32 v72, v73, v72\n\t" \
-	"v_lshlrev_b32_e32 v72, 2, v72\n\t" \
-	"ds_read_b64 v[80:81], v69 offset:0\n\t" \
-	"ds_read_b32 v96, v71 offset:14336\n\t" \
-	"ds_read_b64 v[82:83], v69 offset:8\n\t" \
-	"ds_read_b32 v97, v71 offset:12288\n\t" \
-	"ds_read_b64 v[84:85], v69 offset:16\n\t" \
-	"ds_read_b32 v98, v71 offset:10240\n\t" \
-	"ds_read_b64 v[86:87], v69 offset:24\n\t" \
-	"ds_read_b32 v99, v71 offset:8192\n\t" \
-	"ds_read_b64 v[88:89], v69 offset:32\n\t" \
-	"ds_read_b32 v100, v71 offset:6144\n\t" \
-	"ds_read_b64 v[90:91], v69 offset:40\n\t" \
-	"ds_read_b32 v101, v71 offset:4096\n\t" \
-	"ds_read_b64 v[92:93], v69 offset:48\n\t" \
-	"ds_read_b32 v102, v71 offset:2048\n\t" \
-	"ds_read_b64 v[94:95], v69 offset:56\n\t" \
-	"ds_read_b32 v103, v71 offset:0\n\t" \
+	"v_and_b32_e32 v68, 0xffff, v70\n\t" \
+	"v_lshrrev_b32_e32 v69, 16, v70\n\t" \
+	"ds_read_b32 v72, v68 offset:14336\n\t" \
+	"ds_read_b32 v73, v68 offset:12288\n\t" \
+	"ds_read_b32 v74, v68 offset:10240\n\t" \
+	"ds_read_b32 v75, v68 offset:8192\n\t" \
+	"ds_read_b32 v76, v68 offset:6144\n\t" \
+	"ds_read_b32 v77, v68 offset:4096\n\t" \
+	"ds_read_b32 v78, v68 offset:2048\n\t" \
+	"ds_read_b32 v79, v68 offset:0\n\t" \
+	"ds_read_b32 v80, v69 offset:0\n\t" \
+	"ds_read_b32 v81, v69 offset:2048\n\t" \
+	"ds_read_b32 v82, v69 offset:4096\n\t" \
+	"ds_read_b32 v83, v69 offset:6144\n\t" \
+	"ds_read_b32 v84, v69 offset:8192\n\t" \
+	"ds_read_b32 v85, v69 offset:10240\n\t" \
+	"ds_read_b32 v86, v69 offset:12288\n\t" \
+	"ds_read_b32 v87, v69 offset:14336\n\t" \
+	"s_bitcmp1_b32 s95, 4\n\t" \
+	"s_cbranch_scc1 .Lnb_db_b1\n\t" \
+	"s_waitcnt lgkmcnt(14)\n\t" \
+	"v_pk_fma_f32 v[64:65], v[88:89], v[72:73], v[64:65] op_sel:[0,0,0] op_sel_hi:[1,0,1]\n\t" \
+	"v_pk_fma_f32 v[66:67], v[90:91], v[72:73], v[66:67] op_sel:[0,1,0] op_sel_hi:[1,1,1]\n\t" \
 	"s_waitcnt lgkmcnt(12)\n\t" \
-	"v_pk_fma_f32 v[64:65], v[80:81], v[96:97], v[64:65] op_sel:[0,0,0] op_sel_hi:[1,0,1]\n\t" \
-	"v_pk_fma_f32 v[66:67], v[82:83], v[96:97], v[66:67] op_sel:[0,1,0] op_sel_hi:[1,1,1]\n\t" \
-	"ds_read_b64 v[104:105], v69 offset:64\n\t" \
-	"ds_read_b32 v120, v72 offset:0\n\t" \
-	"ds_read_b64 v[106:107], v69 offset:72\n\t" \
-	"ds_read_b32 v121, v72 offset:2048\n\t" \
+	"v_pk_fma_f32 v[64:65], v[92:93], v[74:75], v[64:65] op_sel:[0,0,0] op_sel_hi:[1,0,1]\n\t" \
+	"v_pk_fma_f32 v[66:67], v[94:95], v[74:75], v[66:67] op_sel:[0,1,0] op_sel_hi:[1,1,1]\n\t" \
+	"s_waitcnt lgkmcnt(10)\n\t" \
+	"v_pk_fma_f32 v[64:65], v[96:97], v[76:77], v[64:65] op_sel:[0,0,0] op_sel_hi:[1,0,1]\n\t" \
+	"v_pk_fma_f32 v[66:67], v[98:99], v[76:77], v[66:67] op_sel:[0,1,0] op_sel_hi:[1,1,1]\n\t" \
+	"s_waitcnt lgkmcnt(8)\n\t" \
+	"v_pk_fma_f32 v[64:65], v[100:101], v[78:79], v[64:65] op_sel:[0,0,0] op_sel_hi:[1,0,1]\n\t" \
+	"v_pk_fma_f32 v[66:67], v[102:103], v[78:79], v[66:67] op_sel:[0,1,0] op_sel_hi:[1,1,1]\n\t" \
+	"s_waitcnt lgkmcnt(6)\n\t" \
+	"v_pk_fma_f32 v[64:65], v[104:105], v[80:81], v[64:65] op_sel:[0,0,0] op_sel_hi:[1,0,1]\n\t" \
+	"v_pk_fma_f32 v[66:67], v[106:107], v[80:81], v[66:67] op_sel:[0,1,0] op_sel_hi:[1,1,1]\n\t" \
+	"s_waitcnt lgkmcnt(4)\n\t" \
+	"v_pk_fma_f32 v[64:65], v[108:109], v[82:83], v[64:65] op_sel:[0,0,0] op_sel_hi:[1,0,1]\n\t" \
+	"v_pk_fma_f32 v[66:67], v[110:111], v[82:83], v[66:67] op_sel:[0,1,0] op_sel_hi:[1,1,1]\n\t" \
+	"s_waitcnt lgkmcnt(2)\n\t" \
+	"v_pk_fma_f32 v[64:65], v[112:113], v[84:85], v[64:65] op_sel:[0,0,0] op_sel_hi:[1,0,1]\n\t" \
+	"v_pk_fma_f32 v[66:67], v[114:115], v[84:85], v[66:67] op_sel:[0,1,0] op_sel_hi:[1,1,1]\n\t" \
+	"s_waitcnt lgkmcnt(0)\n\t" \
+	"v_pk_fma_f32 v[64:65], v[116:117], v[86:87], v[64:65] op_sel:[0,0,0] op_sel_hi:[1,0,1]\n\t" \
+	"v_pk_fma_f32 v[66:67], v[118:119], v[86:87], v[66:67] op_sel:[0,1,0] op_sel_hi:[1,1,1]\n\t" \
+	"s_branch .Lnb_db_sum\n\t" \
+	".Lnb_db_b1:\n\t" \
+	"s_waitcnt lgkmcnt(14)\n\t" \
+	"v_pk_fma_f32 v[64:65], v[90:91], v[72:73], v[64:65] op_sel:[0,0,0] op_sel_hi:[1,0,1]\n\t" \
+	"v_pk_fma_f32 v[66:67], v[92:93], v[72:73], v[66:67] op_sel:[0,1,0] op_sel_hi:[1,1,1]\n\t" \
 	"s_waitcnt lgkmcnt(12)\n\t" \
-	"v_pk_fma_f32 v[64:65], v[84:85], v[98:99], v[64:65] op_sel:[0,0,0] op_sel_hi:[1,0,1]\n\t" \
-	"v_pk_fma_f32 v[66:67], v[86:87], v[98:99], v[66:67] op_sel:[0,1,0] op_sel_hi:[1,1,1]\n\t" \
-	"ds_read_b64 v[108:109], v69 offset:80\n\t" \
-	"ds_read_b32 v122, v72 offset:4096\n\t" \
-	"ds_read_b64 v[110:111], v69 offset:88\n\t" \
-	"ds_read_b32 v123, v72 offset:6144\n\t" \
-	"s_waitcnt lgkmcnt(12)\n\t" \
-	"v_pk_fma_f32 v[64:65], v[88:89], v[100:101], v[64:65] op_sel:[0,0,0] op_sel_hi:[1,0,1]\n\t" \
-	"v_pk_fma_f32 v[66:67], v[90:91], v[100:101], v[66:67] op_sel:[0,1,0] op_sel_hi:[1,1,1]\n\t" \
-	"ds_read_b64 v[112:113], v69 offset:96\n\t" \
-	"ds_read_b32 v124, v72 offset:8192\n\t" \
-	"ds_read_b64 v[114:115], v69 offset:104\n\t" \
-	"ds_read_b32 v125, v72 offset:10240\n\t" \
-	"s_waitcnt lgkmcnt(12)\n\t" \
-	"v_pk_fma_f32 v[64:65], v[92:93], v[102:103], v[64:65] op_sel:[0,0,0] op_sel_hi:[1,0,1]\n\t" \
-	"v_pk_fma_f32 v[66:67], v[94:95], v[102:103], v[66:67] op_sel:[0,1,0] op_sel_hi:[1,1,1]\n\t" \
-	"ds_read_b64 v[116:117], v69 offset:112\n\t" \
-	"ds_read_b32 v126, v72 offset:12288\n\t" \
-	"ds_read_b64 v[118:119], v69 offset:120\n\t" \
-	"ds_read_b32 v127, v72 offset:14336\n\t" \
-	"s_waitcnt lgkmcnt(12)\n\t" \
-	"v_pk_fma_f32 v[64:65], v[104:105], v[120:121], v[64:65] op_sel:[0,0,0] op_sel_hi:[1,0,1]\n\t" \
-	"v_pk_fma_f32 v[66:67], v[106:107], v[120:121], v[66:67] op_sel:[0,1,0] op_sel_hi:[1,1,1]\n\t" \
+	"v_pk_fma_f32 v[64:65], v[94:95], v[74:75], v[64:65] op_sel:[0,0,0] op_sel_hi:[1,0,1]\n\t" \
+	"v_pk_fma_f32 v[66:67], v[96:97], v[74:75], v[66:67] op_sel:[0,1,0] op_sel_hi:[1,1,1]\n\t" \
+	"s_waitcnt lgkmcnt(10)\n\t" \
+	"v_pk_fma_f32 v[64:65], v[98:99], v[76:77], v[64:65] op_sel:[0,0,0] op_sel_hi:[1,0,1]\n\t" \
+	"v_pk_fma_f32 v[66:67], v[100:101], v[76:77], v[66:67] op_sel:[0,1,0] op_sel_hi:[1,1,1]\n\t" \
 	"s_waitcnt lgkmcnt(8)\n\t" \
-	"v_pk_fma_f32 v[64:65], v[108:109], v[122:123], v[64:65] op_sel:[0,0,0] op_sel_hi:[1,0,1]\n\t" \
-	"v_pk_fma_f32 v[66:67], v[110:111], v[122:123], v[66:67] op_sel:[0,1,0] op_sel_hi:[1,1,1]\n\t" \
+	"v_pk_fma_f32 v[64:65], v[102:103], v[78:79], v[64:65] op_sel:[0,0,0] op_sel_hi:[1,0,1]\n\t" \
+	"v_pk_fma_f32 v[66:67], v[104:105], v[78:79], v[66:67] op_sel:[0,1,0] op_sel_hi:[1,1,1]\n\t" \
+	"s_waitcnt lgkmcnt(6)\n\t" \
+	"v_pk_fma_f32 v[64:65], v[106:107], v[80:81], v[64:65] op_sel:[0,0,0] op_sel_hi:[1,0,1]\n\t" \
+	"v_pk_fma_f32 v[66:67], v[108:109], v[80:81], v[66:67] op_sel:[0,1,0] op_sel_hi:[1,1,1]\n\t" \
 	"s_waitcnt lgkmcnt(4)\n\t" \
-	"v_pk_fma_f32 v[64:65], v[112:113], v[124:125], v[64:65] op_sel:[0,0,0] op_sel_hi:[1,0,1]\n\t" \
-	"v_pk_fma_f32 v[66:67], v[114:115], v[124:125], v[66:67] op_sel:[0,1,0] op_sel_hi:[1,1,1]\n\t" \
-	"s_waitcnt lgkmcnt(0)\n\t" \
-	"v_pk_fma_f32 v[64:65], v[116:117], v[126:127], v[64:65] op_sel:[0,0,0] op_sel_hi:[1,0,1]\n\t" \
-	"v_pk_fma_f32 v[66:67], v[118:119], v[126:127], v[66:67] op_sel:[0,1,0] op_sel_hi:[1,1,1]\n\t" \
+	"v_pk_fma_f32 v[64:65], v[110:111], v[82:83], v[64:65] op_sel:[0,0,0] op_sel_hi:[1,0,1]\n\t" \
+	"v_pk_fma_f32 v[66:67], v[112:113], v[82:83], v[66:67] op_sel:[0,1,0] op_sel_hi:[1,1,1]\n\t" \
+	"s_waitcnt lgkmcnt(2)\n\t" \
+	"v_pk_fma_f32 v[64:65], v[114:115], v[84:85], v[64:65] op_sel:[0,0,0] op_sel_hi:[1,0,1]\n\t" \
+	"v_pk_fma_f32 v[66:67], v[116:117], v[84:85], v[66:67] op_sel:[0,1,0] op_sel_hi:[1,1,1]\n\t" \
+	"s_waitcnt lgkmcnt(0)\n\t" \
+	"v_pk_fma_f32 v[64:65], v[118:119], v[86:87], v[64:65] op_sel:[0,0,0] op_sel_hi:[1,0,1]\n\t" \
+	"v_pk_fma_f32 v[66:67], v[120:121], v[86:87], v[66:67] op_sel:[0,1,0] op_sel_hi:[1,1,1]\n\t" \
+	".Lnb_db_sum:\n\t" \
 	"s_mov_b64 exec, -1\n\t" \
 	"v_pk_add_f32 v[74:75], v[64:65], v[66:67]\n\t" \
 	"s_add_u32 s92, %[e], 497\n\t" \
@@ -1403,8 +1394,40 @@
 	"s_bitcmp1_b32 s88, s95\n\t" \
 	"s_addc_u32 s94, s94, s94\n\t" \
 	"s_branch .Lnb_db_walked\n\t" \
+	".Lnb_da_careful:\n\t" \
+	"s_mov_b32 s95, 0\n\t" \
+	"s_lshl1_add_u32 s96, s95, 0\n\t" \
+	"s_bitcmp0_b64 s[90:91], s96\n\t" \
+	"s_cbranch_scc1 .Lnb_db_unsure\n\t" \
+	"s_bitcmp1_b64 s[88:89], s96\n\t" \
+	"s_addc_u32 s95, s95, s95\n\t" \
+	"s_lshl1_add_u32 s96, s95, 2\n\t" \
+	"s_bitcmp0_b64 s[90:91], s96\n\t" \
+	"s_cbranch_scc1 .Lnb_db_unsure\n\t" \
+	"s_bitcmp1_b64 s[88:89], s96\n\t" \
+	"s_addc_u32 s95, s95, s95\n\t" \
+	"s_lshl1_add_u32 s96, s95, 6\n\t" \
+	"s_bitcmp0_b64 s[90:91], s96\n\t" \
+	"s_cbranch_scc1 .Lnb_db_unsure\n\t" \
+	"s_bitcmp1_b64 s[88:89], s96\n\t" \
+	"s_addc_u32 s95, s95, s95\n\t" \
+	"s_lshl1_add_u32 s96, s95, 14\n\t" \
+	"s_bitcmp0_b64 s[90:91], s96\n\t" \
+	"s_cbranch_scc1 .Lnb_db_unsure\n\t" \
+	"s_bitcmp1_b64 s[88:89], s96\n\t" \
+	"s_addc_u32 s95, s95, s95\n\t" \
+	"s_lshl1_add_u32 s96, s95, 30\n\t" \
+	"s_bitcmp0_b64 s[90:91], s96\n\t" \
+	"s_cbranch_scc1 .Lnb_db_unsure\n\t" \
+	"s_bitcmp1_b64 s[88:89], s96\n\t" \
+	"s_addc_u32 s95, s95, s95\n\t" \
+	"s_branch .Lnb_da_walked\n\t" \
 	".Lnb_db_unsure:\n\t" \
 	"s_mov_b32 %[st], 3\n\t" \
+	"s_branch .Lnb_db_end\n\t" \
+	".Lnb_da_wait_end:\n\t" \
+	"s_mov_b64 exec, -1\n\t" \
+	"s_waitcnt lgkmcnt(0)\n\t" \
 	".Lnb_db_end:\n\t"
 #define NB_ASM_TAIL \
 	"v_mov_b32_e32 v65, %[hdrb]\n\t" \
```
